# singer-yang/Aberration-Aware-Depth-from-Focus

Hardware: NVIDIA B200
Metric: focal-stack Mpix*slices/s (fused PSFNet+PSF render) (higher is better)
Workload: dtype fp16 hi/lo split, 3 terms for L1-L7, 2 terms on calibrated fp16 weights for L8, L9 and the head (worst case over any image 7.5e-5), f32 accumulate

## Files before the change

### aberration-aware-depth-from-focus_b200/csrc/aadff_api.cu

```cuda
#include <cuda_fp16.h>
#include <cuda_runtime.h>

#include <atomic>
#include <cmath>
#include <cstdio>
#include <cstring>
#include <mutex>
#include <string>
#include <vector>

#include "../../include/aadff.h"
#include "fused_tc_kernel.cuh"
#include "fused_fast2_kernel.cuh"
#include "gather_kernel.cuh"
#include "gather_coalesced_kernel.cuh"
#include "gather_strip_kernel.cuh"
#include "mlp_fp32_kernel.cuh"
#include "thinlens_kernel.cuh"
#include "focus_kernel.cuh"
#include "psf_conv_kernel.cuh"
#include "train_kernels.cuh"
#include "preprocess_kernel.cuh"
#include "spline_rotate_kernel.cuh"
#include "econ_calib.h"

using namespace aadff;

namespace {

thread_local std::string g_err;
std::atomic<long long> g_launches{0};
std::atomic<int> g_desc_swap{0};
std::atomic<int> g_dbg_flags{0};
std::atomic<unsigned long long*> g_trace{nullptr};

int fail(int code, const std::string& msg) {
    g_err = msg;
    return code;
}

template <int KS, int CN>
void launch_gc(int grid, cudaStream_t st, const float* img, const float* psf, float* out, int N, int C, int H, int W,
               int c0) {
    constexpr int smem = GatherCfg<KS>::SMEM_FLOATS(CN) * (int)sizeof(float);
    if (smem > 48 * 1024)
        cudaFuncSetAttribute(local_psf_coalesced_kernel<KS, CN>, cudaFuncAttributeMaxDynamicSharedMemorySize, smem);
    local_psf_coalesced_kernel<KS, CN><<<grid, GC_WARPS * 32, smem, st>>>(img, psf, out, N, C, H, W, c0);
}
template <int KS>
bool launch_gc_ks(int ks, int cn, int grid, cudaStream_t st, const float* img, const float* psf, float* out, int N, int C,
                  int H, int W, int c0) {
    if constexpr (KS > 31) {
        return false;
    } else {
        if (ks == KS) {
            if (cn == 3) launch_gc<KS, 3>(grid, st, img, psf, out, N, C, H, W, c0);
            else launch_gc<KS, 1>(grid, st, img, psf, out, N, C, H, W, c0);
            return true;
        }
        return launch_gc_ks<KS + 2>(ks, cn, grid, st, img, psf, out, N, C, H, W, c0);
    }
}
bool launch_gather_coalesced(int ks, int cn, int grid, cudaStream_t st, const float* img, const float* psf, float* out,
                             int N, int C, int H, int W, int c0) {
    return launch_gc_ks<3>(ks, cn, grid, st, img, psf, out, N, C, H, W, c0);
}

struct StripShape { int SL, NW, SPX; };
template <int KS> struct StripPlan;
template <> struct StripPlan<3>  { static constexpr StripShape P[3] = {{2, 7, 256}, {2, 12, 128}, {4, 16, 64}}; };
template <> struct StripPlan<5>  { static constexpr StripShape P[3] = {{1, 5, 256}, {2, 6, 128}, {2, 12, 64}}; };
template <> struct StripPlan<7>  { static constexpr StripShape P[3] = {{1, 3, 256}, {1, 6, 128}, {1, 11, 64}}; };
template <> struct StripPlan<9>  { static constexpr StripShape P[3] = {{1, 3, 128}, {1, 7, 64}, {2, 4, 64}}; };
template <> struct StripPlan<11> { static constexpr StripShape P[3] = {{1, 5, 64}, {2, 3, 64}, {2, 3, 64}}; };
template <> struct StripPlan<13> { static constexpr StripShape P[3] = {{2, 2, 64}, {1, 4, 64}, {1, 4, 64}}; };
template <> struct StripPlan<15> { static constexpr StripShape P[3] = {{1, 3, 64}, {3, 1, 64}, {3, 1, 64}}; };
constexpr int STRIP_MAX_KS = 15;

template <int KS, int CN, int SL, int NW, int SPX>
void launch_gs(int sms, cudaStream_t st, const float* img, const float* psf, float* out, int N, int C, int H, int W,
               int c0) {
    constexpr int smem = StripCfg<KS, CN, SPX>::SMEM_BYTES(SL, NW);
    static_assert(smem <= 232448, "strip gather: shared memory plan does not fit");
    if (smem > 48 * 1024)
        cudaFuncSetAttribute(local_psf_strip_kernel<KS, CN, SL, NW, SPX>, cudaFuncAttributeMaxDynamicSharedMemorySize, smem);
    const long long rows = (long long)N * ((W + SPX - 1) / SPX) * H;
    const int grid = (int)std::min<long long>((rows + NW - 1) / NW, sms);
    local_psf_strip_kernel<KS, CN, SL, NW, SPX><<<grid, NW * 32, smem, st>>>(img, psf, out, N, C, H, W, c0);
}
template <int KS, int I>
void launch_gs_plan(int cn, int sms, cudaStream_t st, const float* img, const float* psf, float* out, int N, int C, int H,
                    int W, int c0) {
    constexpr StripShape S = StripPlan<KS>::P[I];
    if (cn == 3) launch_gs<KS, 3, S.SL, S.NW, S.SPX>(sms, st, img, psf, out, N, C, H, W, c0);
    else launch_gs<KS, 1, S.SL, S.NW, S.SPX>(sms, st, img, psf, out, N, C, H, W, c0);
}
template <int KS>
bool launch_gs_ks(int ks, int cn, int plan, int sms, cudaStream_t st, const float* img, const float* psf, float* out,
                  int N, int C, int H, int W, int c0) {
    if constexpr (KS > STRIP_MAX_KS) {
        return false;
    } else {
        if (ks == KS) {
            if (plan < 0) {
                plan = 2;
                for (int i = 0; i < 3; ++i) {
                    const int spx = StripPlan<KS>::P[i].SPX;
                    if ((long long)((W + spx - 1) / spx) * spx * 10 <= (long long)W * 11 || spx <= GSW_PX) { plan = i; break; }
                }
            }
            if (plan == 1) launch_gs_plan<KS, 1>(cn, sms, st, img, psf, out, N, C, H, W, c0);
            else if (plan == 2) launch_gs_plan<KS, 2>(cn, sms, st, img, psf, out, N, C, H, W, c0);
            else launch_gs_plan<KS, 0>(cn, sms, st, img, psf, out, N, C, H, W, c0);
            return true;
        }
        return launch_gs_ks<KS + 2>(ks, cn, plan, sms, st, img, psf, out, N, C, H, W, c0);
    }
}

template <int KS>
bool launch_psf_conv(int ks, int grid, cudaStream_t st, const PsfConvArgs& a) {
    if constexpr (KS > 31) {
        return false;
    } else {
        if (ks == KS) {
            psf_conv_kernel<KS><<<grid, PC_NT, 0, st>>>(a);
            return true;
        }
        return launch_psf_conv<KS + 2>(ks, grid, st, a);
    }
}

template <int KS>
bool launch_thinlens(int ks, int grid, int smem, cudaStream_t st, const ThinLensArgs& a, const CUtensorMap& map) {
    if constexpr (KS > 31) {
        return false;
    } else {
        if (ks == KS) {
            if (smem > 48 * 1024)
                cudaFuncSetAttribute(thinlens_render_kernel<KS>, cudaFuncAttributeMaxDynamicSharedMemorySize, smem);
            thinlens_render_kernel<KS><<<grid, TL_NT, smem, st>>>(a, map);
            return true;
        }
        return launch_thinlens<KS + 2>(ks, grid, smem, st, a, map);
    }
}
template <int KS>
bool thinlens2_geometry(int ks, int cn, int* box_w, int* box_h, int* smem) {
    if constexpr (KS > 31) {
        return false;
    } else {
        if (ks == KS) {
            *box_w = ThinLens2Cfg<KS>::BW;
            *box_h = ThinLens2Cfg<KS>::HH;
            *smem = ThinLens2Cfg<KS>::SMEM_BYTES(cn);
            return true;
        }
        return thinlens2_geometry<KS + 2>(ks, cn, box_w, box_h, smem);
    }
}
template <int KS>
bool launch_thinlens2(int ks, int grid, int smem, cudaStream_t st, const ThinLensArgs& a, const CUtensorMap& map) {
    if constexpr (KS > 31) {
        return false;
    } else {
        if (ks == KS) {
            if (smem > 48 * 1024)
                cudaFuncSetAttribute(thinlens_render2_kernel<KS>, cudaFuncAttributeMaxDynamicSharedMemorySize, smem);
            thinlens_render2_kernel<KS><<<grid, TL_NT, smem, st>>>(a, map);
            return true;
        }
        return launch_thinlens2<KS + 2>(ks, grid, smem, st, a, map);
    }
}

typedef CUresult (*EncodeTiledFn)(CUtensorMap*, CUtensorMapDataType, cuuint32_t, void*, const cuuint64_t*, const cuuint64_t*,
                                  const cuuint32_t*, const cuuint32_t*, CUtensorMapInterleave, CUtensorMapSwizzle,
                                  CUtensorMapL2promotion, CUtensorMapFloatOOBfill);
EncodeTiledFn encode_tiled_fn() {
    static EncodeTiledFn fn = []() -> EncodeTiledFn {
        void* p = nullptr;
        cudaDriverEntryPointQueryResult q;
        if (cudaGetDriverEntryPoint("cuTensorMapEncodeTiled", &p, cudaEnableDefault, &q) != cudaSuccess ||
            q != cudaDriverEntryPointSuccess)
            return nullptr;
        return reinterpret_cast<EncodeTiledFn>(p);
    }();
    return fn;
}

bool make_image_map(CUtensorMap* map, const float* img, long long planes, int H, int W, int box_w, int box_h, int box_c) {
    EncodeTiledFn enc = encode_tiled_fn();
    if (!enc || (W % 4) != 0 || (reinterpret_cast<uintptr_t>(img) % 16) != 0 || box_w > 256 || box_h > 256 || box_c > 256)
        return false;
    const cuuint64_t dims[3] = {(cuuint64_t)W, (cuuint64_t)H, (cuuint64_t)planes};
    const cuuint64_t strides[2] = {(cuuint64_t)W * 4, (cuuint64_t)W * H * 4};
    const cuuint32_t box[3] = {(cuuint32_t)box_w, (cuuint32_t)box_h, (cuuint32_t)box_c};
    const cuuint32_t estr[3] = {1, 1, 1};
    return enc(map, CU_TENSOR_MAP_DATA_TYPE_FLOAT32, 3, const_cast<float*>(img), dims, strides, box, estr,
               CU_TENSOR_MAP_INTERLEAVE_NONE, CU_TENSOR_MAP_SWIZZLE_NONE, CU_TENSOR_MAP_L2_PROMOTION_L2_128B,
               CU_TENSOR_MAP_FLOAT_OOB_FILL_NONE) == CUDA_SUCCESS;
}

#define CUDA_TRY(expr)                                                                          \
    do {                                                                                        \
        cudaError_t _e = (expr);                                                                \
        if (_e != cudaSuccess)                                                                  \
            return fail(AADFF_E_CUDA, std::string(#expr) + ": " + cudaGetErrorString(_e));      \
    } while (0)

struct DeviceGuard {
    int prev = -1;
    bool ok = true;
    explicit DeviceGuard(int dev) {
        if (cudaGetDevice(&prev) != cudaSuccess) { ok = false; return; }
        if (prev != dev && cudaSetDevice(dev) != cudaSuccess) ok = false;
    }
    ~DeviceGuard() {
        if (prev >= 0) cudaSetDevice(prev);
    }
};

template <typename T>
int upload(const std::vector<T>& h, T** d) {
    CUDA_TRY(cudaMalloc(reinterpret_cast<void**>(d), h.size() * sizeof(T)));
    CUDA_TRY(cudaMemcpy(*d, h.data(), h.size() * sizeof(T), cudaMemcpyHostToDevice));
    return AADFF_OK;
}

void pack_group(const float* W, int out_f, int in_f, int n0, int N, std::vector<__half>& dst) {
    for (int kc = 0; kc < in_f / TC_SLAB_K; ++kc) {
        for (int part = 0; part < 2; ++part) {
            const size_t base = dst.size();
            dst.resize(base + (size_t)N * TC_SLAB_K);
            for (int k = 0; k < TC_SLAB_K; ++k) {
                for (int n = 0; n < N; ++n) {
                    const int row = n0 + n, col = kc * TC_SLAB_K + k;
                    const float w = (row < out_f) ? W[(size_t)row * in_f + col] : 0.0f;
                    const __half hi = __float2half_rn(w);
                    const __half v = part == 0 ? hi : __float2half_rn(w - __half2float(hi));
                    dst[base + (size_t)(k / 8) * (N * 8) + (size_t)n * 8 + (k % 8)] = v;
                }
            }
        }
    }
}

void pack_bias_slab(const float* bias, int N, std::vector<__half>& dst) {
    const size_t base = dst.size();
    dst.resize(base + (size_t)N * 16, __float2half_rn(0.f));
    for (int n = 0; n < N; ++n) {
        const __half hi = __float2half_rn(bias[n]);
        dst[base + (size_t)n * 8 + 0] = hi;
        dst[base + (size_t)n * 8 + 1] = __float2half_rn(bias[n] - __half2float(hi));
    }
}

}

struct aadff_psfnet {
    int device = 0, ks = 0, kk = 0, n_layers = 0;
    int num_sms = 0, smem_optin = 0;
    Fp32Net f32{};
    std::vector<float*> owned;
    bool tc_ok = false;
    std::string tc_why;
    uint8_t* d_wpack = nullptr;
    float* d_bias_tc = nullptr;
    float* d_w0b0 = nullptr;
    TcGroup groups[TC_MAX_GROUPS]{};
    uint32_t w_off_econ[TC_MAX_GROUPS]{};
    uint8_t* d_wpack_econ = nullptr;
    size_t pack_bytes = 0;
    bool econ_ready = false;
    std::mutex econ_mu;
    std::vector<std::vector<float>> host_w, host_b;
    std::vector<int> host_dims;
    int n_groups = 0, n_hidden = 0, n_bias = 0, head_bias0 = 0;
    cudaStream_t ws_stream = nullptr, ws_copy_stream = nullptr;
    std::vector<cudaEvent_t> ws_events;
    float* ws = nullptr;
    size_t ws_bytes = 0;
};

struct aadff_trainer {
    int device = 0, n_layers = 0, batch = 0, kk = 0;
    std::vector<int> dims;
    std::vector<size_t> w_off, b_off;
    size_t n_params = 0;
    float *params = nullptr, *grads = nullptr, *m = nullptr, *v = nullptr;
    std::vector<float*> act;
    float *z = nullptr, *p = nullptr, *target = nullptr, *loss = nullptr;
    std::vector<float*> dz;
    AdamHyper* hyper = nullptr;
    AdamHyper host_hyper{};
    long long step = 0;
    cudaGraph_t graph = nullptr;
    cudaGraphExec_t exec = nullptr;
    cudaStream_t cap_stream = nullptr;
    cudaStream_t side[2] = {nullptr, nullptr};
    std::vector<cudaEvent_t> evs;
};

static void trainer_free(aadff_trainer* t) {
    if (!t) return;
    DeviceGuard guard(t->device);
    if (t->exec) cudaGraphExecDestroy(t->exec);
    if (t->graph) cudaGraphDestroy(t->graph);
    if (t->cap_stream) cudaStreamDestroy(t->cap_stream);
    for (cudaEvent_t ev : t->evs) cudaEventDestroy(ev);
    for (int i = 0; i < 2; ++i) if (t->side[i]) cudaStreamDestroy(t->side[i]);
    for (float* a : t->act) cudaFree(a);
    cudaFree(t->params); cudaFree(t->grads); cudaFree(t->m); cudaFree(t->v);
    cudaFree(t->z); cudaFree(t->p); cudaFree(t->target);
    for (float* d : t->dz) cudaFree(d);
    cudaFree(t->loss); cudaFree(t->hyper);
    delete t;
}

template <int EPI>
static void tg_launch(cudaStream_t st, const float* A, long long sa_i, long long sa_k, const float* B, long long sb_k,
                      long long sb_j, float* C, int M, int N, int K, const float* aux) {
    dim3 grid((N + TG_TILE - 1) / TG_TILE, (M + TG_TILE - 1) / TG_TILE);
    train_gemm_kernel<EPI><<<grid, TG_NT, 0, st>>>(A, sa_i, sa_k, B, sb_k, sb_j, C, M, N, K, aux);
}

static int trainer_record(aadff_trainer* t, cudaStream_t st) {
    const int L = t->n_layers, M = t->batch;
    cudaStream_t* side = t->side;
    size_t next_ev = 0;
    auto new_event = [&]() { return t->evs[next_ev++]; };
    for (int l = 0; l < L; ++l) {
        const int K = t->dims[l], N = t->dims[l + 1];
        const float* W = t->params + t->w_off[l];
        const float* b = t->params + t->b_off[l];
        if (l < L - 1) tg_launch<TG_BIAS_RELU>(st, t->act[l], K, 1, W, 1, K, t->act[l + 1], M, N, K, b);
        else tg_launch<TG_BIAS>(st, t->act[l], K, 1, W, 1, K, t->z, M, N, K, b);
    }
    train_head_kernel<<<(M * 32 + 255) / 256, 256, 0, st>>>(t->z, t->target, t->p, t->dz[L - 1], t->loss, M, t->kk);
    for (int l = L - 1; l >= 0; --l) {
        const int K = t->dims[l], N = t->dims[l + 1];
        const float* W = t->params + t->w_off[l];
        const float* dZ = t->dz[l];
        cudaEvent_t ready = new_event();
        cudaEventRecord(ready, st);
        cudaStreamWaitEvent(side[0], ready, 0);
        cudaStreamWaitEvent(side[1], ready, 0);
        tg_launch<TG_PLAIN>(side[0], dZ, 1, N, t->act[l], K, 1, t->grads + t->w_off[l], N, K, M, nullptr);
        train_colsum_kernel<<<(N + 255) / 256, 256, 0, side[1]>>>(dZ, t->grads + t->b_off[l], M, N);
        if (l > 0) tg_launch<TG_RELU_MASK>(st, dZ, N, 1, W, K, 1, t->dz[l - 1], M, K, N, t->act[l]);
    }
    for (int i = 0; i < 2; ++i) {
        cudaEvent_t done = new_event();
        cudaEventRecord(done, side[i]);
        cudaStreamWaitEvent(st, done, 0);
    }
    train_adamw_kernel<<<(int)std::min<size_t>((t->n_params + 255) / 256, 1184), 256, 0, st>>>(
        t->params, t->grads, t->m, t->v, (long long)t->n_params, t->hyper);
    const cudaError_t e = cudaGetLastError();
    if (e != cudaSuccess) return fail(AADFF_E_CUDA, std::string("trainer_record: ") + cudaGetErrorString(e));
    return AADFF_OK;
}


extern "C" {

int aadff_version(void) { return AADFF_VERSION; }
const char* aadff_last_error(void) { return g_err.c_str(); }
int64_t aadff_launch_count(void) { return g_launches.load(); }
int aadff_debug_set_desc_swap(int swap) {
    g_desc_swap.store(swap ? 1 : 0);
    return AADFF_OK;
}

int aadff_debug_set_trace(void* device_buffer) {
    g_trace.store(static_cast<unsigned long long*>(device_buffer));
    return AADFF_OK;
}
int aadff_debug_trace_entries(void) { return TC_TRACE_N; }
int aadff_debug_set_flags(int flags) {
    g_dbg_flags.store(flags);
    return AADFF_OK;
}

int aadff_psfnet_create(const float* const* weights, const float* const* biases, const int* dims, int n_layers,
                        int ks, int device, aadff_psfnet_t* out) {
    if (!weights || !biases || !dims || !out) return fail(AADFF_E_INVALID, "null argument");
    if (n_layers < 2 || n_layers > MAX_LAYERS) return fail(AADFF_E_INVALID, "n_layers must be in [2,16]");
    if (ks < 1 || (ks % 2) == 0) return fail(AADFF_E_INVALID, "kernel size must be odd and positive");
    if (dims[0] != 4 || dims[n_layers] != ks * ks)
        return fail(AADFF_E_INVALID, "dims must start with 4 and end with ks*ks");
    for (int l = 0; l < n_layers; ++l) {
        if (!weights[l] || !biases[l]) return fail(AADFF_E_INVALID, "null layer pointer");
        if (dims[l + 1] < 1 || (l + 1 < n_layers && (dims[l + 1] > 256 || dims[l + 1] % 8)))
            return fail(AADFF_E_INVALID, "hidden widths must be multiples of 8 and <= 256");
    }
    DeviceGuard guard(device);
    if (!guard.ok) return fail(AADFF_E_CUDA, "cannot select CUDA device " + std::to_string(device));
    cudaDeviceProp prop;
    CUDA_TRY(cudaGetDeviceProperties(&prop, device));
    if (prop.major != 10)
        return fail(AADFF_E_CUDA, "libaadff is built for sm_100a only; device is sm_" + std::to_string(prop.major) +
                                      std::to_string(prop.minor));

    aadff_psfnet* h = new aadff_psfnet();
    h->device = device;
    h->ks = ks;
    h->kk = ks * ks;
    h->n_layers = n_layers;
    h->num_sms = prop.multiProcessorCount;
    h->smem_optin = (int)prop.sharedMemPerBlockOptin;

    h->f32.n_layers = n_layers;
    h->f32.kk = h->kk;
    for (int l = 0; l < n_layers; ++l) {
        const int K = dims[l], Nf = dims[l + 1], npad = (Nf + 7) / 8 * 8;
        std::vector<float> wt((size_t)K * npad, 0.f), b(npad, 0.f);
        for (int n = 0; n < Nf; ++n) {
            b[n] = biases[l][n];
            for (int k = 0; k < K; ++k) wt[(size_t)k * npad + n] = weights[l][(size_t)n * K + k];
        }
        float *dw = nullptr, *db = nullptr;
        int rc = upload(wt, &dw);
        if (rc) { aadff_psfnet_destroy(h); return rc; }
        h->owned.push_back(dw);
        rc = upload(b, &db);
        if (rc) { aadff_psfnet_destroy(h); return rc; }
        h->owned.push_back(db);
        h->f32.wt[l] = dw;
        h->f32.bias[l] = db;
        h->f32.k[l] = K;
        h->f32.npad[l] = npad;
    }
#define CREATE_TRY(expr)                                                                         \
    do {                                                                                         \
        cudaError_t _e = (expr);                                                                 \
        if (_e != cudaSuccess) {                                                                 \
            aadff_psfnet_destroy(h);                                                             \
            return fail(AADFF_E_CUDA, std::string(#expr) + ": " + cudaGetErrorString(_e));       \
        }                                                                                        \
    } while (0)
    CREATE_TRY(cudaFuncSetAttribute(mlp_fp32_kernel<true>, cudaFuncAttributeMaxDynamicSharedMemorySize, F32_SMEM));
    CREATE_TRY(cudaFuncSetAttribute(mlp_fp32_kernel<false>, cudaFuncAttributeMaxDynamicSharedMemorySize, F32_SMEM));

    h->tc_ok = true;
    if (n_layers < 3 || dims[1] != 64) { h->tc_ok = false; h->tc_why = "first hidden width must be 64"; }
    for (int l = 2; l < n_layers && h->tc_ok; ++l)
        if (dims[l] != TC_HID) { h->tc_ok = false; h->tc_why = "hidden width must be 256"; }
    if (ks > TC_MAX_KS) { h->tc_ok = false; h->tc_why = "kernel size > 31"; }
    const int nh_pad = (h->kk + 15) / 16 * 16;
    const int n_head_blocks = (nh_pad + 255) / 256;
    if (h->tc_ok && (n_layers - 2) + n_head_blocks > TC_MAX_GROUPS) { h->tc_ok = false; h->tc_why = "too many layers"; }
    if (h->tc_ok) {
        std::vector<__half> pack;
        std::vector<float> bias_tc;
        int gi = 0;
        for (int l = 1; l < n_layers - 1; ++l, ++gi) {
            TcGroup& g = h->groups[gi];
            g.w_off = (uint32_t)(pack.size() * sizeof(__half));
            g.K = (uint16_t)dims[l];
            g.N = TC_HID;
            g.terms = 3;
            g.bias_off = (uint16_t)bias_tc.size();
            g.new_a = 1;
            g.tap0 = 0;
            pack_bias_slab(biases[l], TC_HID, pack);
            pack_group(weights[l], dims[l + 1], dims[l], 0, TC_HID, pack);
            bias_tc.insert(bias_tc.end(), biases[l], biases[l] + TC_HID);
        }
        h->n_hidden = gi;
        const int L = n_layers - 1;
        const int head_bias0 = (int)bias_tc.size();
        h->head_bias0 = head_bias0;
        bias_tc.resize(head_bias0 + nh_pad, 0.f);
        for (int n = 0; n < h->kk; ++n) bias_tc[head_bias0 + n] = -1.4426950408889634f * biases[L][n];
        for (int b = 0; b < n_head_blocks; ++b, ++gi) {
            TcGroup& g = h->groups[gi];
            const int N = std::min(256, nh_pad - 256 * b);
            g.w_off = (uint32_t)(pack.size() * sizeof(__half));
            g.K = TC_HID;
            g.N = (uint16_t)N;
            g.terms = 3;
            g.bias_off = (uint16_t)(head_bias0 + 256 * b);
            g.new_a = (b == 0);
            g.tap0 = (uint16_t)(256 * b);
            pack_group(weights[L], h->kk, TC_HID, 256 * b, N, pack);
        }
        h->n_groups = gi;
        h->n_bias = (int)bias_tc.size();
        h->host_dims.assign(dims, dims + n_layers + 1);
        for (int l = 0; l < n_layers; ++l) {
            h->host_w.emplace_back(weights[l], weights[l] + (size_t)dims[l] * dims[l + 1]);
            h->host_b.emplace_back(biases[l], biases[l] + dims[l + 1]);
        }
        h->pack_bytes = pack.size() * sizeof(__half);
        std::vector<float> w0b0(320);
        std::memcpy(w0b0.data(), weights[0], 256 * sizeof(float));
        std::memcpy(w0b0.data() + 256, biases[0], 64 * sizeof(float));
        __half* dp = nullptr;
        int rc = upload(pack, &dp);
        if (rc) { aadff_psfnet_destroy(h); return rc; }
        h->d_wpack = reinterpret_cast<uint8_t*>(dp);
        rc = upload(bias_tc, &h->d_bias_tc);
        if (rc) { aadff_psfnet_destroy(h); return rc; }
        rc = upload(w0b0, &h->d_w0b0);
        if (rc) { aadff_psfnet_destroy(h); return rc; }
        const int so = h->smem_optin;
        const auto attr = cudaFuncAttributeMaxDynamicSharedMemorySize;
        CREATE_TRY(cudaFuncSetAttribute(fused_psfnet_render_kernel<true, false, 0>, attr, so));
#define AADFF_SET_ATTR(U)                                                                        \
        CREATE_TRY(cudaFuncSetAttribute(fused_psfnet_render_kernel<false, false, U>, attr, so));   \
        CREATE_TRY(cudaFuncSetAttribute(fused_psfnet_render_kernel<false, false, U, true>, attr, so));   \
        CREATE_TRY(cudaFuncSetAttribute(fused_psfnet_render_kernel<false, true, U>, attr, so));
        AADFF_SET_ATTR(0) AADFF_SET_ATTR(1) AADFF_SET_ATTR(3) AADFF_SET_ATTR(13) AADFF_SET_ATTR(12) AADFF_SET_ATTR(15)
#undef AADFF_SET_ATTR
        CREATE_TRY(cudaFuncSetAttribute(fused_psfnet_render_kernel<false, false, 14>, attr, so));
        CREATE_TRY(cudaFuncSetAttribute(fused_psfnet_render_kernel<false, true, 14>, attr, so));
    }
#undef CREATE_TRY
    *out = h;
    return AADFF_OK;
}

int aadff_psfnet_destroy(aadff_psfnet_t h) {
    if (!h) return AADFF_OK;
    DeviceGuard guard(h->device);
    for (float* p : h->owned) cudaFree(p);
    cudaFree(h->d_wpack);
    cudaFree(h->d_wpack_econ);
    cudaFree(h->d_bias_tc);
    cudaFree(h->d_w0b0);
    cudaFree(h->ws);
    if (h->ws_stream) cudaStreamDestroy(h->ws_stream);
    if (h->ws_copy_stream) cudaStreamDestroy(h->ws_copy_stream);
    for (cudaEvent_t e : h->ws_events) cudaEventDestroy(e);
    delete h;
    return AADFF_OK;
}

static int ensure_econ(aadff_psfnet_t h) {
    std::lock_guard<std::mutex> lock(h->econ_mu);
    if (h->econ_ready) return AADFF_OK;
    const int n_layers = h->n_layers, L = n_layers - 1;
    std::vector<const float*> W(n_layers), B(n_layers);
    for (int l = 0; l < n_layers; ++l) { W[l] = h->host_w[l].data(); B[l] = h->host_b[l].data(); }
    std::vector<std::vector<float>> wq;
    calibrate_econ(W.data(), B.data(), h->host_dims.data(), n_layers, TC_ECON_FIRST_LAYER, wq);
    std::vector<__half> pack;
    for (int g2 = 0; g2 < h->n_groups; ++g2) {
        const bool hidden = g2 < h->n_hidden;
        const int l = hidden ? g2 + 1 : L;
        h->w_off_econ[g2] = h->groups[g2].w_off;
        if (l < TC_ECON_FIRST_LAYER || wq[l].empty()) continue;
        h->w_off_econ[g2] = (uint32_t)(h->pack_bytes + pack.size() * sizeof(__half));
        if (hidden) {
            pack_bias_slab(B[l], TC_HID, pack);
            pack_group(wq[l].data(), h->host_dims[l + 1], h->host_dims[l], 0, TC_HID, pack);
        } else {
            pack_group(wq[l].data(), h->kk, TC_HID, h->groups[g2].tap0, h->groups[g2].N, pack);
        }
    }
    uint8_t* d = nullptr;
    CUDA_TRY(cudaMalloc(reinterpret_cast<void**>(&d), h->pack_bytes + pack.size() * sizeof(__half)));
    cudaError_t e = cudaMemcpy(d, h->d_wpack, h->pack_bytes, cudaMemcpyDeviceToDevice);
    if (e == cudaSuccess) e = cudaMemcpy(d + h->pack_bytes, pack.data(), pack.size() * sizeof(__half), cudaMemcpyHostToDevice);
    if (e != cudaSuccess) {
        cudaFree(d);
        return fail(AADFF_E_CUDA, std::string("econ weight upload: ") + cudaGetErrorString(e));
    }
    h->d_wpack_econ = d;
    h->econ_ready = true;
    return AADFF_OK;
}

static int launch_fast2(aadff_psfnet_t h, const RenderArgs& ra, cudaStream_t st, long long tile_row0, long long tile_row1) {
    if (!h->tc_ok || h->n_groups != h->n_hidden + 1 || !(g_dbg_flags.load() & 32)) return 1;
    F2Params P{};
    P.ra = ra;
    P.wpack = h->d_wpack;
    P.bias = h->d_bias_tc;
    P.w0b0 = h->d_w0b0;
    P.n_groups = h->n_groups;
    P.n_hidden = h->n_hidden;
    P.n_bias = h->n_bias;
    P.bias_skip = h->head_bias0;
    P.kk = h->kk;
    for (int i = 0; i < h->n_groups; ++i) { P.g[i] = h->groups[i]; P.g[i].terms = 1; }
    P.tiles_x = (ra.W + TC_TILE_W - 1) / TC_TILE_W;
    P.tiles_y = (ra.H + TC_TILE_H - 1) / TC_TILE_H;
    P.n_tiles = (long long)P.tiles_x * P.tiles_y * ra.N * ra.S;
    if (tile_row1 >= 0) {
        P.tile0 = tile_row0 * P.tiles_x;
        P.n_tiles = (tile_row1 - tile_row0) * P.tiles_x;
        if (P.n_tiles <= 0) return AADFF_OK;
    }
    P.halo_pitch = TC_TILE_W + ra.ks - 1;
    P.halo_bytes = (uint32_t)(TC_TILE_H + ra.ks - 1) * P.halo_pitch * 16;
    const uint32_t bias_bytes = (uint32_t)(h->n_bias - h->head_bias0) * 4;
    P.off_stage = 2 * TC_A_PART_BYTES;
    P.off_bias = P.off_stage + F2_STAGES * TC_STAGE_BYTES;
    P.off_w0 = P.off_bias + bias_bytes;
    P.off_halo = (P.off_w0 + 320 * 4 + 15u) & ~15u;
    P.off_red = P.off_halo + 2 * P.halo_bytes;
    P.off_bar = P.off_red + 2 * TC_M * 5 * 4;
    P.off_ones = (P.off_bar + TC_BAR_BYTES + 15u) & ~15u;
    P.off_bslab = P.off_ones + 2 * TC_A_LBO;
    const uint32_t smem = P.off_bslab + 2 * TC_BSLAB_BYTES;
    if (smem > (uint32_t)h->smem_optin) return 1;
    const long long units = (P.n_tiles + 1) / 2;
    const int grid = (int)std::min<long long>(units, h->num_sms);
    cudaFuncSetAttribute(fused_fast2_kernel, cudaFuncAttributeMaxDynamicSharedMemorySize, h->smem_optin);
    fused_fast2_kernel<<<grid, TC_NT, smem, st>>>(P);
    g_launches.fetch_add(1);
    CUDA_TRY(cudaGetLastError());
    return AADFF_OK;
}

static int launch_tc(aadff_psfnet_t h, RenderArgs ra, int mode, cudaStream_t st, long long tile_row0 = 0,
                     long long tile_row1 = -1, const float* probes = nullptr, float* psf_out = nullptr,
                     long long n_probes = 0) {
    if (!h->tc_ok) return fail(AADFF_E_UNSUPPORTED, "tensor-core path unavailable: " + h->tc_why + " (use AADFF_MODE_FP32)");
    const bool econ_like = (mode == AADFF_MODE_ECON || mode == AADFF_MODE_ECON8);
    if (econ_like) {
        const int rc = ensure_econ(h);
        if (rc) return rc;
    }
    if (mode == AADFF_MODE_FAST && probes == nullptr && g_trace.load() == nullptr) {
        const int rc = launch_fast2(h, ra, st, tile_row0, tile_row1);
        if (rc <= 0) return rc;
    }
    TcParams P{};
    P.ra = ra;
    P.wpack = econ_like ? h->d_wpack_econ : h->d_wpack;
    P.bias = h->d_bias_tc;
    P.w0b0 = h->d_w0b0;
    P.n_groups = h->n_groups;
    P.n_hidden = h->n_hidden;
    P.n_bias = h->n_bias;
    P.bias_skip = h->head_bias0;
    P.kk = h->kk;
    const int econ_first_dbg = (g_dbg_flags.load() >> 16) & 15;
    const int econ_first = (econ_first_dbg > TC_ECON_FIRST_GROUP) ? econ_first_dbg : TC_ECON_FIRST_GROUP;
    for (int i = 0; i < h->n_groups; ++i) {
        P.g[i] = h->groups[i];
        const bool hidden = i < h->n_hidden;
        P.g[i].terms = (mode == AADFF_MODE_FAST) ? 1
                       : (mode == AADFF_MODE_MIXED && i >= TC_MIXED_FIRST_GROUP) ? 1
                       : (mode == AADFF_MODE_ECON && i >= econ_first) ? 2
                       : (mode == AADFF_MODE_ECON8 && i >= TC_ECON8_FIRST_GROUP) ? 2
                       : 3;
        if (econ_like && P.g[i].terms == 2 && !(g_dbg_flags.load() & 256))
            P.g[i].w_off = h->w_off_econ[i];
        (void)hidden;
    }
    P.tiles_x = (ra.W + TC_TILE_W - 1) / TC_TILE_W;
    P.tiles_y = (ra.H + TC_TILE_H - 1) / TC_TILE_H;
    P.n_tiles = (long long)P.tiles_x * P.tiles_y * ra.N * ra.S;
    if (tile_row1 >= 0) {
        P.tile0 = tile_row0 * P.tiles_x;
        P.n_tiles = (tile_row1 - tile_row0) * P.tiles_x;
        if (P.n_tiles <= 0) return AADFF_OK;
    }
    if (probes != nullptr) {
        P.probes = probes;
        P.psf_out = psf_out;
        P.n_probes = n_probes;
        P.n_tiles = (n_probes + TC_M - 1) / TC_M;
    }
    P.trace = g_trace.load();
    P.dbg = (uint32_t)g_dbg_flags.load();
    uint32_t halo_bytes = (uint32_t)(TC_TILE_H + ra.ks - 1) * TC_HALO_PITCH * 16;
    if (probes != nullptr) halo_bytes = std::max<uint32_t>(halo_bytes, 8 * 32 * 9 * 4);
    const uint32_t bias_bytes = (uint32_t)(h->n_bias - h->head_bias0) * 4;
    const uint32_t ones_bytes = 2 * TC_A_LBO;
    const uint32_t bslab_bytes = 2 * TC_BSLAB_BYTES;
    const uint32_t fixed = 2 * TC_A_PART_BYTES + bias_bytes + 320 * 4 + halo_bytes + TC_M * 5 * 4 + TC_BAR_BYTES + ones_bytes +
                           bslab_bytes + 16;
    int stages = 4;
    while (stages >= 2 && fixed + (uint32_t)stages * TC_STAGE_BYTES > (uint32_t)h->smem_optin) --stages;
    if (stages < 2) return fail(AADFF_E_UNSUPPORTED, "shared memory budget exceeded for this kernel size / channel count");
    bool any_lo = false;
    for (int i = 0; i < h->n_groups; ++i) any_lo |= (P.g[i].terms >= 2);
    P.off_stage = 2 * TC_A_PART_BYTES;
    P.off_bias = P.off_stage + stages * TC_STAGE_BYTES;
    P.off_w0 = P.off_bias + bias_bytes;
    P.off_halo = P.off_w0 + 320 * 4;
    P.off_red = P.off_halo + halo_bytes;
    P.off_bar = P.off_red + TC_M * 5 * 4;
    P.off_ones = (P.off_bar + TC_BAR_BYTES + 15u) & ~15u;
    P.off_bslab = P.off_ones + ones_bytes;
    const uint32_t smem = P.off_bslab + bslab_bytes;
    P.kslab = (!any_lo && stages == 4) ? 2 : 1;
    P.n_stages = (P.kslab == 2) ? 4 : stages;
    int grid = (int)std::min<long long>(P.n_tiles, h->num_sms);
    bool all3 = true, all1 = true, econ_pat = true, econ8_pat = true, mixed_pat = true, aligned = (P.n_stages == 4 && P.kslab == 1);
    for (int i = 0; i < h->n_groups; ++i) {
        const int t = P.g[i].terms;
        all3 &= (t == 3);
        all1 &= (t == 1);
        econ_pat &= (t == (i < TC_ECON_FIRST_GROUP ? 3 : 2));
        econ8_pat &= (t == (i < TC_ECON8_FIRST_GROUP ? 3 : 2));
        mixed_pat &= (t == (i < TC_MIXED_FIRST_GROUP ? 3 : 1));
        aligned &= (((P.g[i].K / TC_SLAB_K) * (t == 3 ? 2 : 1)) % 4 == 0);
    }
    static_assert(TC_ECON_FIRST_GROUP == TC_ECON_FIRST_LAYER - 1, "group g holds layer g + 1");
    int uni = 0;
    if (all3 && P.kslab == 1) uni = aligned ? 13 : 3;
    else if (all1 && P.kslab == 2) uni = 1;
    else if (econ_pat && aligned) uni = 12;
    else if (econ8_pat && aligned && h->n_groups > TC_ECON8_FIRST_GROUP) uni = 14;
    else if (mixed_pat && aligned) uni = 15;
    const bool cl2 = P.probes == nullptr && P.trace == nullptr && uni != 0 && uni != 14 && (P.dbg & 8u) && h->num_sms >= 2;
    if (cl2) {
        grid = (int)std::min<long long>((P.n_tiles + 1) & ~1ll, (long long)(h->num_sms & ~1));
        cudaLaunchConfig_t cfg{};
        cfg.gridDim = dim3((unsigned)grid);
        cfg.blockDim = dim3(TC_NT);
        cfg.dynamicSmemBytes = smem;
        cfg.stream = st;
        cudaLaunchAttribute la[1];
        la[0].id = cudaLaunchAttributeClusterDimension;
        la[0].val.clusterDim.x = 2; la[0].val.clusterDim.y = 1; la[0].val.clusterDim.z = 1;
        cfg.attrs = la;
        cfg.numAttrs = 1;
        cudaError_t le = cudaSuccess;
        switch (uni) {
            case 1: le = cudaLaunchKernelEx(&cfg, fused_psfnet_render_kernel<false, false, 1, true>, P); break;
            case 3: le = cudaLaunchKernelEx(&cfg, fused_psfnet_render_kernel<false, false, 3, true>, P); break;
            case 13: le = cudaLaunchKernelEx(&cfg, fused_psfnet_render_kernel<false, false, 13, true>, P); break;
            case 12: le = cudaLaunchKernelEx(&cfg, fused_psfnet_render_kernel<false, false, 12, true>, P); break;
            default: le = cudaLaunchKernelEx(&cfg, fused_psfnet_render_kernel<false, false, 15, true>, P); break;
        }
        if (le != cudaSuccess) return fail(AADFF_E_CUDA, std::string("cluster launch: ") + cudaGetErrorString(le));
    } else if (P.trace != nullptr && P.probes == nullptr) {
        fused_psfnet_render_kernel<true, false, 0><<<grid, TC_NT, smem, st>>>(P);
    } else {
#define AADFF_LAUNCH(U)                                                                                   \
        case U:                                                                                           \
            if (P.probes != nullptr) fused_psfnet_render_kernel<false, true, U><<<grid, TC_NT, smem, st>>>(P);   \
            else fused_psfnet_render_kernel<false, false, U><<<grid, TC_NT, smem, st>>>(P);               \
            break;
        switch (uni) {
            AADFF_LAUNCH(1) AADFF_LAUNCH(3) AADFF_LAUNCH(13) AADFF_LAUNCH(12) AADFF_LAUNCH(14) AADFF_LAUNCH(15)
            default:
                if (P.probes != nullptr) fused_psfnet_render_kernel<false, true, 0><<<grid, TC_NT, smem, st>>>(P);
                else fused_psfnet_render_kernel<false, false, 0><<<grid, TC_NT, smem, st>>>(P);
        }
#undef AADFF_LAUNCH
    }
    g_launches.fetch_add(1);
    CUDA_TRY(cudaGetLastError());
    return AADFF_OK;
}

static int render_stack_impl(aadff_psfnet_t h, const float* img, const float* depth, const float* foc, int foc_stride,
                             float* out, const int64_t out_strides[5], int N, int C, int S, int H, int W, float d_min,
                             float d_max, int mode, void* stream, long long tile_row0 = 0, long long tile_row1 = -1);

int aadff_tile_row_height(void) { return TC_TILE_H; }
int aadff_econ_first_group(void) { return TC_ECON_FIRST_GROUP; }

int aadff_render_stack_rows_f32(aadff_psfnet_t h, const float* img, const float* depth, const float* foc, float* out,
                                const int64_t out_strides[5], int N, int C, int S, int H, int W, float d_min,
                                float d_max, int mode, int64_t tile_row_begin, int64_t tile_row_end, void* stream) {
    const long long total = (long long)N * S * ((H + TC_TILE_H - 1) / TC_TILE_H);
    if (tile_row_begin < 0 || tile_row_end < tile_row_begin || tile_row_end > total)
        return fail(AADFF_E_INVALID, "tile-row range outside [0, N*S*ceil(H/8)]");
    return render_stack_impl(h, img, depth, foc, S, out, out_strides, N, C, S, H, W, d_min, d_max, mode, stream,
                             tile_row_begin, tile_row_end);
}

int aadff_render_stack_f32(aadff_psfnet_t h, const float* img, const float* depth, const float* foc, float* out,
                           const int64_t out_strides[5], int N, int C, int S, int H, int W, float d_min,
                           float d_max, int mode, void* stream) {
    return render_stack_impl(h, img, depth, foc, S, out, out_strides, N, C, S, H, W, d_min, d_max, mode, stream);
}

static int render_stack_impl(aadff_psfnet_t h, const float* img, const float* depth, const float* foc, int foc_stride,
                             float* out, const int64_t out_strides[5], int N, int C, int S, int H, int W, float d_min,
                             float d_max, int mode, void* stream, long long tile_row0, long long tile_row1) {
    if (!h || !img || !depth || !foc || !out || !out_strides) return fail(AADFF_E_INVALID, "null argument");
    if (N < 0 || C < 1 || S < 1 || H < 1 || W < 1) return fail(AADFF_E_INVALID, "bad shape");
    if (mode < 0 || mode > 5) return fail(AADFF_E_INVALID, "unknown mode");
    if (d_max == d_min) return fail(AADFF_E_INVALID, "d_max == d_min");
    if (N == 0) return AADFF_OK;
    DeviceGuard guard(h->device);
    if (!guard.ok) return fail(AADFF_E_CUDA, "cannot select device");
    cudaStream_t st = static_cast<cudaStream_t>(stream);
    RenderArgs ra{};
    ra.img = img; ra.depth = depth; ra.foc = foc; ra.out = out;
    ra.os_n = out_strides[0]; ra.os_c = out_strides[1]; ra.os_s = out_strides[2];
    ra.os_h = out_strides[3]; ra.os_w = out_strides[4];
    ra.N = N; ra.S = S; ra.H = H; ra.W = W; ra.ks = h->ks; ra.Ctot = C;
    ra.foc_stride = foc_stride;
    ra.d_min = d_min;
    ra.d_range = d_max - d_min;
    ra.step_x = (W > 1) ? (1.0f - (-1.0f)) / (float)(W - 1) : 0.f;
    ra.step_y = (H > 1) ? (-1.0f - 1.0f) / (float)(H - 1) : 0.f;
    for (int c0 = 0; c0 < C; c0 += 4) {
        ra.c0 = c0;
        ra.C = std::min(4, C - c0);
        if (mode == AADFF_MODE_FP32) {
            long long M0 = 0, M = (long long)N * S * H * W;
            if (tile_row1 >= 0) {
                const long long tiles_y = (H + TC_TILE_H - 1) / TC_TILE_H;
                auto flat_row = [&](long long R) { return (R / tiles_y) * H + std::min<long long>((R % tiles_y) * TC_TILE_H, H); };
                M0 = flat_row(tile_row0) * W;
                M = flat_row(tile_row1) * W;
            }
            if (M > M0) {
                const int grid = (int)std::min<long long>((M - M0 + F32_TP - 1) / F32_TP, (long long)h->num_sms * 8);
                mlp_fp32_kernel<true><<<grid, F32_NT, F32_SMEM, st>>>(h->f32, ra, nullptr, nullptr, M0, M);
                g_launches.fetch_add(1);
                CUDA_TRY(cudaGetLastError());
            }
        } else {
            int rc = launch_tc(h, ra, mode, st, tile_row0, tile_row1);
            if (rc) return rc;
        }
    }
    return AADFF_OK;
}

int aadff_render_stack_host_f32(aadff_psfnet_t h, const float* img, const float* depth, const float* foc,
                                float* out, int N, int C, int S, int H, int W, float d_min, float d_max, int mode) {
    if (!h || !img || !depth || !foc || !out) return fail(AADFF_E_INVALID, "null argument");
    if (N < 1 || C < 1 || S < 1 || H < 1 || W < 1) return fail(AADFF_E_INVALID, "bad shape");
    DeviceGuard guard(h->device);
    if (!guard.ok) return fail(AADFF_E_CUDA, "cannot select device");
    const size_t n_img = (size_t)N * C * H * W, n_dep = (size_t)N * H * W, n_foc = (size_t)N * S;
    const size_t n_out = n_img * S;
    auto up = [](size_t n) { return (n + 63) / 64 * 64; };
    const size_t need = (up(n_img) + up(n_dep) + up(n_foc) + up(n_out)) * sizeof(float);
    if (!h->ws_stream) CUDA_TRY(cudaStreamCreateWithFlags(&h->ws_stream, cudaStreamNonBlocking));
    if (need > h->ws_bytes) {
        if (h->ws) CUDA_TRY(cudaFree(h->ws));
        h->ws = nullptr;
        h->ws_bytes = 0;
        CUDA_TRY(cudaMalloc(reinterpret_cast<void**>(&h->ws), need));
        h->ws_bytes = need;
    }
    float* d_img = h->ws;
    float* d_dep = d_img + up(n_img);
    float* d_foc = d_dep + up(n_dep);
    float* d_out = d_foc + up(n_foc);
    cudaStream_t st = h->ws_stream;
    CUDA_TRY(cudaMemcpyAsync(d_img, img, n_img * sizeof(float), cudaMemcpyHostToDevice, st));
    CUDA_TRY(cudaMemcpyAsync(d_dep, depth, n_dep * sizeof(float), cudaMemcpyHostToDevice, st));
    CUDA_TRY(cudaMemcpyAsync(d_foc, foc, n_foc * sizeof(float), cudaMemcpyHostToDevice, st));
    const int64_t strides[5] = {(int64_t)C * S * H * W, (int64_t)S * H * W, (int64_t)H * W, W, 1};
    if (!h->ws_copy_stream) CUDA_TRY(cudaStreamCreateWithFlags(&h->ws_copy_stream, cudaStreamNonBlocking));
    if (h->ws_events.size() < (size_t)S) {
        const size_t old = h->ws_events.size();
        h->ws_events.resize(S);
        for (size_t i = old; i < (size_t)S; ++i) CUDA_TRY(cudaEventCreateWithFlags(&h->ws_events[i], cudaEventDisableTiming));
    }
    const size_t plane = (size_t)H * W * sizeof(float);
    for (int s = 0; s < S; ++s) {
        int rc = render_stack_impl(h, d_img, d_dep, d_foc + s, S, d_out + (size_t)s * H * W, strides, N, C, 1, H, W, d_min,
                                   d_max, mode, st);
        if (rc) return rc;
        CUDA_TRY(cudaEventRecord(h->ws_events[s], st));
        CUDA_TRY(cudaStreamWaitEvent(h->ws_copy_stream, h->ws_events[s], 0));
        for (int n = 0; n < N; ++n) {
            const size_t off = ((size_t)n * C * S + s) * H * W;
            CUDA_TRY(cudaMemcpy2DAsync(out + off, (size_t)S * plane, d_out + off, (size_t)S * plane, plane, C,
                                       cudaMemcpyDeviceToHost, h->ws_copy_stream));
        }
    }
    CUDA_TRY(cudaStreamSynchronize(h->ws_copy_stream));
    CUDA_TRY(cudaStreamSynchronize(st));
    return AADFF_OK;
}

int aadff_psfnet_pred_f32(aadff_psfnet_t h, const float* inp, float* psf, int64_t M, void* stream) {
    if (!h || !inp || !psf) return fail(AADFF_E_INVALID, "null argument");
    if (M < 0) return fail(AADFF_E_INVALID, "negative M");
    if (M == 0) return AADFF_OK;
    DeviceGuard guard(h->device);
    if (!guard.ok) return fail(AADFF_E_CUDA, "cannot select device");
    RenderArgs ra{};
    ra.ks = h->ks;
    const int grid = (int)std::min<long long>((M + F32_TP - 1) / F32_TP, (long long)h->num_sms * 8);
    mlp_fp32_kernel<false><<<grid, F32_NT, F32_SMEM, static_cast<cudaStream_t>(stream)>>>(h->f32, ra, inp, psf, 0, M);
    g_launches.fetch_add(1);
    CUDA_TRY(cudaGetLastError());
    return AADFF_OK;
}

int aadff_psfnet_pred_tc_f32(aadff_psfnet_t h, const float* inp, float* psf, int64_t M, int mode, void* stream) {
    if (!h || !inp || !psf) return fail(AADFF_E_INVALID, "null argument");
    if (M < 0) return fail(AADFF_E_INVALID, "negative M");
    if (mode == AADFF_MODE_FP32) return aadff_psfnet_pred_f32(h, inp, psf, M, stream);
    if (mode < 0 || mode > 5) return fail(AADFF_E_INVALID, "unknown mode");
    if (reinterpret_cast<uintptr_t>(inp) % 16) return fail(AADFF_E_INVALID, "inp must be 16-byte aligned");
    if (M == 0) return AADFF_OK;
    DeviceGuard guard(h->device);
    if (!guard.ok) return fail(AADFF_E_CUDA, "cannot select device");
    RenderArgs ra{};
    ra.ks = h->ks; ra.N = 1; ra.S = 1; ra.H = 1; ra.W = 1; ra.C = 1; ra.Ctot = 1;
    return launch_tc(h, ra, mode, static_cast<cudaStream_t>(stream), 0, -1, inp, psf, (long long)M);
}

int aadff_local_psf_render_f32(const float* img, const float* psf, float* out, int N, int C, int H, int W, int ks,
                               void* stream) {
    if (!img || !psf || !out) return fail(AADFF_E_INVALID, "null argument");
    if (N < 0 || C < 1 || H < 1 || W < 1) return fail(AADFF_E_INVALID, "bad shape");
    if (ks < 1 || (ks % 2) == 0) return fail(AADFF_E_INVALID, "kernel size must be odd and positive");
    if (N == 0) return AADFF_OK;
    int dev = 0, sms = 0;
    CUDA_TRY(cudaGetDevice(&dev));
    CUDA_TRY(cudaDeviceGetAttribute(&sms, cudaDevAttrMultiProcessorCount, dev));
    cudaStream_t st = static_cast<cudaStream_t>(stream);
    const int dbg = g_dbg_flags.load();
    if (ks >= 3 && ks <= STRIP_MAX_KS && !(dbg & (128 | 512)) && W % 4 == 0 && reinterpret_cast<uintptr_t>(psf) % 16 == 0 &&
        reinterpret_cast<uintptr_t>(out) % 8 == 0 && (long long)N * H * ((W + 31) / 32) < (1ll << 40)) {
        int c0 = 0;
        while (c0 < C) {
            const int cn = (C - c0 >= 3) ? 3 : 1;
            if (!launch_gs_ks<3>(ks, cn, (dbg & 1024) ? 1 : (dbg & 4096) ? 2 : (dbg & 8192) ? 0 : -1, sms, st, img, psf, out, N, C, H, W, c0))
                return fail(AADFF_E_INVALID, "unsupported kernel size");
            g_launches.fetch_add(1);
            CUDA_TRY(cudaGetLastError());
            c0 += cn;
        }
        return AADFF_OK;
    }
    if (ks >= 3 && ks <= 31 && !(g_dbg_flags.load() & 128)) {
        const long long tiles = (long long)N * ((H + GC_WARPS - 1) / GC_WARPS) * ((W + GC_TW - 1) / GC_TW);
        if (tiles >= (1ll << 31)) return fail(AADFF_E_INVALID, "image batch too large for one launch");
        const int grid = (int)std::min<long long>(tiles, sms);
        int c0 = 0;
        while (c0 < C) {
            const int cn = (C - c0 >= 3) ? 3 : 1;
            if (!launch_gather_coalesced(ks, cn, grid, st, img, psf, out, N, C, H, W, c0))
                return fail(AADFF_E_INVALID, "unsupported kernel size");
            g_launches.fetch_add(1);
            CUDA_TRY(cudaGetLastError());
            c0 += cn;
        }
        return AADFF_OK;
    }
    const int kk = ks * ks;
    int P = 32;
    while (P > 4 && P * kk * 4 > GS_BUF_BYTES) P >>= 1;
    const bool stream_ok = (W % 4 == 0) && (reinterpret_cast<uintptr_t>(psf) % 16 == 0) && (P * kk * 4 <= GS_BUF_BYTES);
    if (stream_ok) {
        const int nbuf = (P == 32 && (g_dbg_flags.load() & 64)) ? 2 : 1;
        const int nw = (nbuf == 2) ? GS_TILE_H_2BUF : GS_TILE_H_1BUF;
        const int buf_bytes = (P * kk * 4 + 127) / 128 * 128;
        const int HH = nw + ks - 1, pitch = (GS_TILE_W + ks - 1) | 1;
        const int smem = nw * nbuf * buf_bytes + GS_MAXC * HH * pitch * 4 + 16 * nw;
        if (smem > 48 * 1024) {
            if (nw == GS_TILE_H_1BUF)
                CUDA_TRY(cudaFuncSetAttribute(local_psf_stream_kernel<GS_TILE_H_1BUF>,
                                              cudaFuncAttributeMaxDynamicSharedMemorySize, smem));
            else
                CUDA_TRY(cudaFuncSetAttribute(local_psf_stream_kernel<GS_TILE_H_2BUF>,
                                              cudaFuncAttributeMaxDynamicSharedMemorySize, smem));
        }
        const long long tiles = (long long)N * ((H + nw - 1) / nw) * ((W + GS_TILE_W - 1) / GS_TILE_W);
        const int grid = (int)std::min<long long>(tiles, sms);
        for (int c0 = 0; c0 < C; c0 += GS_MAXC) {
            const int cn = std::min(GS_MAXC, C - c0);
            if (nw == GS_TILE_H_1BUF)
                local_psf_stream_kernel<GS_TILE_H_1BUF><<<grid, nw * 32, smem, st>>>(img, psf, out, N, C, H, W, ks, c0, cn,
                                                                                   P, nbuf, buf_bytes);
            else
                local_psf_stream_kernel<GS_TILE_H_2BUF><<<grid, nw * 32, smem, st>>>(img, psf, out, N, C, H, W, ks, c0, cn,
                                                                                   P, nbuf, buf_bytes);
            g_launches.fetch_add(1);
            CUDA_TRY(cudaGetLastError());
        }
        return AADFF_OK;
    }
    const int smem = GATHER_WARPS * 32 * (GATHER_TT + 1) * (int)sizeof(float);
    if (smem > 48 * 1024)
        CUDA_TRY(cudaFuncSetAttribute(local_psf_render_kernel, cudaFuncAttributeMaxDynamicSharedMemorySize, smem));
    const long long items = (long long)N * H * ((W + 31) / 32);
    const int grid = (int)std::min<long long>((items + GATHER_WARPS - 1) / GATHER_WARPS, (long long)sms * 3);
    for (int c0 = 0; c0 < C; c0 += GATHER_MAXC) {
        local_psf_render_kernel<<<grid, GATHER_WARPS * 32, smem, st>>>(img, psf, out, N, C, H, W, ks, c0,
                                                                       std::min(GATHER_MAXC, C - c0));
        g_launches.fetch_add(1);
        CUDA_TRY(cudaGetLastError());
    }
    return AADFF_OK;
}

int aadff_any_negative_f32(const float* x, int64_t n, unsigned char* flag_dev, void* stream) {
    if (!x || !flag_dev || n < 0) return fail(AADFF_E_INVALID, "bad argument");
    cudaStream_t st = static_cast<cudaStream_t>(stream);
    CUDA_TRY(cudaMemsetAsync(flag_dev, 0, 1, st));
    if (n == 0) return AADFF_OK;
    const int grid = (int)std::min<long long>((n + 255) / 256, 592);
    any_negative_kernel<<<grid, 256, 0, st>>>(x, (long long)n, flag_dev);
    g_launches.fetch_add(1);
    CUDA_TRY(cudaGetLastError());
    return AADFF_OK;
}

int aadff_thinlens_render_f32(const float* img, const float* depth, const float* foc, float* out, int N, int C, int H,
                              int W, int ks, float foc_len, float fnum, float pixel_size, float d_lo, float d_hi,
                              int flip_sign, const unsigned char* flip_sign_dev, void* stream) {
    if (!img || !depth || !foc || !out) return fail(AADFF_E_INVALID, "null argument");
    if (N < 0 || C < 1 || H < 1 || W < 1) return fail(AADFF_E_INVALID, "bad shape");
    if (ks < 1 || (ks % 2) == 0) return fail(AADFF_E_INVALID, "kernel size must be odd and positive");
    if (!(fnum > 0.f) || !(pixel_size > 0.f) || !(d_hi > d_lo)) return fail(AADFF_E_INVALID, "bad lens parameters");
    if (N == 0) return AADFF_OK;
    int dev = 0, sms = 0, optin = 0;
    CUDA_TRY(cudaGetDevice(&dev));
    CUDA_TRY(cudaDeviceGetAttribute(&sms, cudaDevAttrMultiProcessorCount, dev));
    CUDA_TRY(cudaDeviceGetAttribute(&optin, cudaDevAttrMaxSharedMemoryPerBlockOptin, dev));
    ThinLensArgs a{};
    a.img = img; a.depth = depth; a.foc = foc; a.out = out;
    a.N = N; a.C = C; a.H = H; a.W = W;
    a.k1 = (float)((double)foc_len / (double)fnum);
    a.foc_len = foc_len; a.ps = pixel_size; a.d_lo = d_lo; a.d_hi = d_hi; a.flip = flip_sign ? 1 : 0;
    a.flip_dev = flip_sign_dev;
    if (ks > 31) return fail(AADFF_E_UNSUPPORTED, "thin-lens kernel sizes above 31 are not built");
    cudaStream_t st = static_cast<cudaStream_t>(stream);
    const bool two_px = !(g_dbg_flags.load() & 2048);
    const int tl_r = (ks - 1) / 2, tl_sh = (4 - tl_r % 4) % 4;
    const int tile_w = two_px ? TL2_TILE_W : TL_TILE_W;
    const long long tiles = (long long)N * ((H + TL_TILE_H - 1) / TL_TILE_H) * ((W + tile_w - 1) / tile_w);
    if (tiles >= (1ll << 31)) return fail(AADFF_E_INVALID, "image batch too large for one launch");
    const int grid = (int)std::min<long long>(tiles, (long long)sms * 4);
    for (int c0 = 0; c0 < C; c0 += TL_MAXC) {
        a.c0 = c0;
        a.cn = std::min(TL_MAXC, C - c0);
        int HH = TL_TILE_H + ks - 1, BW = (TL_TILE_W + ks - 1 + tl_sh + 3) / 4 * 4;
        int smem = (ks <= 15 ? 2 : 1) * ((a.cn * HH * BW + 31) / 32 * 32) * 4 + 128;
        if (two_px && !thinlens2_geometry<1>(ks, a.cn, &BW, &HH, &smem)) return fail(AADFF_E_INVALID, "unsupported kernel size");
        if (smem > optin) return fail(AADFF_E_UNSUPPORTED, "kernel size too large for the shared-memory halo tile");
        CUtensorMap map;
        std::memset(&map, 0, sizeof(map));
        a.use_tma = make_image_map(&map, img, (long long)N * C, H, W, BW, HH, a.cn) && !(g_dbg_flags.load() & 16);
        const bool launched = two_px ? launch_thinlens2<1>(ks, grid, smem, st, a, map) : launch_thinlens<1>(ks, grid, smem, st, a, map);
        if (!launched) return fail(AADFF_E_INVALID, "unsupported kernel size");
        g_launches.fetch_add(1);
        CUDA_TRY(cudaGetLastError());
    }
    return AADFF_OK;
}

int aadff_render_psf_map_f32(const float* img, const float* psf_map, float* out, int B, int C, int H, int W, int ks,
                             int grid, const int* row_bounds, const int* col_bounds, void* stream) {
    if (!img || !psf_map || !out || !row_bounds || !col_bounds) return fail(AADFF_E_INVALID, "null argument");
    if (B < 0 || C < 1 || H < 1 || W < 1) return fail(AADFF_E_INVALID, "bad shape");
    if (ks < 1 || ks > 31 || (ks % 2) == 0) return fail(AADFF_E_INVALID, "PSF kernel size should be odd (and <= 31)");
    if (grid < 1 || grid > PC_MAX_GRID) return fail(AADFF_E_INVALID, "grid must be in [1, 32]");
    if ((ks - 1) / 2 >= H || (ks - 1) / 2 >= W) return fail(AADFF_E_INVALID, "reflect padding needs (ks-1)/2 < H, W");
    if (B == 0) return AADFF_OK;
    PsfConvArgs a{};
    a.img = img; a.psf_map = psf_map; a.out = out;
    a.B = B; a.C = C; a.H = H; a.W = W; a.grid = grid;
    for (int i = 0; i <= grid; ++i) { a.hb[i] = row_bounds[i]; a.wb[i] = col_bounds[i]; }
    if (a.hb[0] != 0 || a.wb[0] != 0 || a.hb[grid] > H || a.wb[grid] > W) return fail(AADFF_E_INVALID, "bad patch bounds");
    for (int i = 0; i < grid; ++i) {
        if (a.hb[i + 1] < a.hb[i] || a.wb[i + 1] < a.wb[i]) return fail(AADFF_E_INVALID, "patch bounds must ascend");
        a.max_ch = std::max(a.max_ch, a.hb[i + 1] - a.hb[i]);
        a.max_cw = std::max(a.max_cw, a.wb[i + 1] - a.wb[i]);
    }
    if (a.max_ch == 0 || a.max_cw == 0) return AADFF_OK;
    int dev = 0, sms = 0;
    CUDA_TRY(cudaGetDevice(&dev));
    CUDA_TRY(cudaDeviceGetAttribute(&sms, cudaDevAttrMultiProcessorCount, dev));
    const long long tiles = (long long)B * C * grid * grid * ((a.max_ch + PC_TILE_H - 1) / PC_TILE_H) *
                            ((a.max_cw + PC_TILE_W - 1) / PC_TILE_W);
    const int nblk = (int)std::min<long long>(tiles, (long long)sms * 8);
    if (!launch_psf_conv<1>(ks, nblk, static_cast<cudaStream_t>(stream), a)) return fail(AADFF_E_INVALID, "unsupported kernel size");
    g_launches.fetch_add(1);
    CUDA_TRY(cudaGetLastError());
    return AADFF_OK;
}

int aadff_preprocess_rgbd_u8(const uint8_t* bgr, const uint16_t* depth, float* aif_out, float* depth_out, int B, int H, int W,
                             int h, int w, float depth_div, int depth_mode, const float* jitter, const uint8_t* flips,
                             void* stream) {
    if ((!bgr && !depth) || (bgr && !aif_out) || (depth && !depth_out)) return fail(AADFF_E_INVALID, "null argument");
    if (B < 0 || H < 1 || W < 1 || h < 1 || w < 1) return fail(AADFF_E_INVALID, "bad shape");
    if (depth && !(depth_div > 0.f)) return fail(AADFF_E_INVALID, "depth divisor must be positive");
    if (depth_mode != 0 && depth_mode != 1) return fail(AADFF_E_INVALID, "depth_mode must be 0 (antialias) or 1 (cv2 linear)");
    if (B == 0) return AADFF_OK;
    PreprocessArgs a{};
    a.bgr = bgr; a.depth = depth; a.aif_out = bgr ? aif_out : nullptr; a.depth_out = depth ? depth_out : nullptr;
    a.jitter = jitter; a.flips = flips;
    a.B = B; a.H = H; a.W = W; a.h = h; a.w = w; a.depth_div = depth_div; a.depth_mode = depth_mode;
    const long long per_image = (long long)h * w;
    const dim3 grid((unsigned)std::min<long long>((per_image + 255) / 256, 148 * 16), (unsigned)B);
    if (B > 65535) return fail(AADFF_E_INVALID, "batch too large for one launch");
    preprocess_rgbd_kernel<false><<<grid, 256, 0, static_cast<cudaStream_t>(stream)>>>(a);
    g_launches.fetch_add(1);
    CUDA_TRY(cudaGetLastError());
    return AADFF_OK;
}

int aadff_prepare_planes_u8(const uint8_t* bgr, const uint16_t* depth, float* planes, int B, int H, int W, float depth_div,
                            const float* jitter, const uint8_t* flips, void* stream) {
    if ((!bgr && !depth) || !planes) return fail(AADFF_E_INVALID, "null argument");
    if (B < 0 || H < 1 || W < 1) return fail(AADFF_E_INVALID, "bad shape");
    if (depth && !(depth_div > 0.f)) return fail(AADFF_E_INVALID, "depth divisor must be positive");
    if (B > 65535) return fail(AADFF_E_INVALID, "batch too large for one launch");
    if (B == 0) return AADFF_OK;
    PlanesArgs a{};
    a.bgr = bgr; a.depth = depth; a.planes = planes; a.jitter = jitter; a.flips = flips;
    a.B = B; a.H = H; a.W = W; a.P = (bgr ? 3 : 0) + (depth ? 1 : 0); a.depth_div = depth_div;
    const dim3 grid((unsigned)std::min<long long>(((long long)H * W + 255) / 256, 148 * 8), (unsigned)B);
    prepare_planes_kernel<<<grid, 256, 0, static_cast<cudaStream_t>(stream)>>>(a);
    g_launches.fetch_add(1);
    CUDA_TRY(cudaGetLastError());
    return AADFF_OK;
}

int aadff_spline_affine_f32(const float* planes, float* work, float* out, int B, int P, int H, int W, const double* xform,
                            int clamp_plane, void* stream) {
    if (!planes || !work || !out || !xform) return fail(AADFF_E_INVALID, "null argument");
    if (B < 0 || P < 1 || H < 1 || W < 1) return fail(AADFF_E_INVALID, "bad shape");
    if (clamp_plane >= P) return fail(AADFF_E_INVALID, "clamp_plane out of range");
    if (B > 65535) return fail(AADFF_E_INVALID, "batch too large for one launch");
    if (B == 0) return AADFF_OK;
    cudaStream_t st = static_cast<cudaStream_t>(stream);
    const long long n = (long long)B * P * H * W;
    float* tmp = work;
    float* coef = work + n;
    const unsigned blocks = (unsigned)std::min<long long>((n + 255) / 256, 148 * 16);
    spline_prefilter_kernel<1><<<blocks, 256, 0, st>>>(planes, tmp, (long long)B * P, H, W);
    spline_prefilter_kernel<0><<<blocks, 256, 0, st>>>(tmp, coef, (long long)B * P, H, W);
    AffineArgs a{};
    a.coef = coef; a.raw = planes; a.out = out; a.xform = xform; a.B = B; a.P = P; a.H = H; a.W = W; a.clamp_plane = clamp_plane;
    const dim3 grid((unsigned)std::min<long long>(((long long)H * W + 255) / 256, 148 * 8), (unsigned)B);
    spline_affine_kernel<<<grid, 256, 0, st>>>(a);
    g_launches.fetch_add(3);
    CUDA_TRY(cudaGetLastError());
    return AADFF_OK;
}

int aadff_resize_planes_f32(const float* planes, float* aif_out, float* depth_out, int B, int P, int H, int W, int h, int w,
                            int depth_mode, void* stream) {
    if (!planes || (!aif_out && !depth_out)) return fail(AADFF_E_INVALID, "null argument");
    if (B < 0 || H < 1 || W < 1 || h < 1 || w < 1) return fail(AADFF_E_INVALID, "bad shape");
    if (P != (aif_out ? 3 : 0) + (depth_out ? 1 : 0)) return fail(AADFF_E_INVALID, "P must be 3 (image), 1 (depth) or 4 (both)");
    if (depth_mode != 0 && depth_mode != 1) return fail(AADFF_E_INVALID, "depth_mode must be 0 (antialias) or 1 (cv2 linear)");
    if (B > 65535) return fail(AADFF_E_INVALID, "batch too large for one launch");
    if (B == 0) return AADFF_OK;
    PreprocessArgs a{};
    a.aif_out = aif_out; a.depth_out = depth_out; a.fsrc = planes; a.fsrc_planes = P; a.fsrc_depth_plane = P - 1;
    a.B = B; a.H = H; a.W = W; a.h = h; a.w = w; a.depth_div = 1.f; a.depth_mode = depth_mode;
    const long long per_image = (long long)h * w;
    const dim3 grid((unsigned)std::min<long long>((per_image + 255) / 256, 148 * 16), (unsigned)B);
    preprocess_rgbd_kernel<true><<<grid, 256, 0, static_cast<cudaStream_t>(stream)>>>(a);
    g_launches.fetch_add(1);
    CUDA_TRY(cudaGetLastError());
    return AADFF_OK;
}

int aadff_select_focus_f32(const float* depth_m, int B, int64_t HW, int num, float* out, void* stream) {
    if (!depth_m || !out) return fail(AADFF_E_INVALID, "null argument");
    if (B < 0 || HW < 1) return fail(AADFF_E_INVALID, "bad shape");
    if (num <= 3) return fail(AADFF_E_INVALID, "Focal stack size is too small");
    if (B == 0) return AADFF_OK;
    select_focus_kernel<<<B, FOCUS_NT, 0, static_cast<cudaStream_t>(stream)>>>(depth_m, (long long)HW, num, out);
    g_launches.fetch_add(1);
    CUDA_TRY(cudaGetLastError());
    return AADFF_OK;
}


int aadff_trainer_create(const float* const* weights, const float* const* biases, const int* dims, int n_layers,
                         int batch, float beta1, float beta2, float eps, float weight_decay, int device,
                         aadff_trainer_t* out) {
    if (!weights || !biases || !dims || !out) return fail(AADFF_E_INVALID, "null argument");
    if (n_layers < 1 || n_layers > MAX_LAYERS || batch < 1) return fail(AADFF_E_INVALID, "bad n_layers / batch");
    DeviceGuard guard(device);
    if (!guard.ok) return fail(AADFF_E_CUDA, "cannot select CUDA device " + std::to_string(device));
    aadff_trainer* t = new aadff_trainer();
    t->device = device; t->n_layers = n_layers; t->batch = batch; t->kk = dims[n_layers];
    t->dims.assign(dims, dims + n_layers + 1);
    t->host_hyper.beta1 = beta1; t->host_hyper.beta2 = beta2; t->host_hyper.eps = eps; t->host_hyper.weight_decay = weight_decay;
    size_t off = 0;
    int wmax = 0;
    for (int l = 0; l < n_layers; ++l) {
        t->w_off.push_back(off); off += (size_t)dims[l] * dims[l + 1];
        t->b_off.push_back(off); off += (size_t)dims[l + 1];
        wmax = std::max(wmax, std::max(dims[l], dims[l + 1]));
    }
    t->n_params = off;
#define TR_TRY(expr)                                                                             \
    do {                                                                                         \
        cudaError_t _e = (expr);                                                                 \
        if (_e != cudaSuccess) {                                                                 \
            trainer_free(t);                                                                     \
            return fail(AADFF_E_CUDA, std::string(#expr) + ": " + cudaGetErrorString(_e));       \
        }                                                                                        \
    } while (0)
    auto dalloc = [&](float** p, size_t n) { return cudaMalloc(reinterpret_cast<void**>(p), n * sizeof(float)); };
    TR_TRY(dalloc(&t->params, off)); TR_TRY(dalloc(&t->grads, off)); TR_TRY(dalloc(&t->m, off)); TR_TRY(dalloc(&t->v, off));
    TR_TRY(cudaMemset(t->m, 0, off * sizeof(float))); TR_TRY(cudaMemset(t->v, 0, off * sizeof(float)));
    for (int l = 0; l < n_layers; ++l) {
        if (!weights[l] || !biases[l]) { trainer_free(t); return fail(AADFF_E_INVALID, "null layer pointer"); }
        TR_TRY(cudaMemcpy(t->params + t->w_off[l], weights[l], (size_t)dims[l] * dims[l + 1] * sizeof(float), cudaMemcpyHostToDevice));
        TR_TRY(cudaMemcpy(t->params + t->b_off[l], biases[l], (size_t)dims[l + 1] * sizeof(float), cudaMemcpyHostToDevice));
        float* a = nullptr;
        TR_TRY(dalloc(&a, (size_t)batch * dims[l]));
        t->act.push_back(a);
    }
    TR_TRY(dalloc(&t->z, (size_t)batch * t->kk)); TR_TRY(dalloc(&t->p, (size_t)batch * t->kk));
    TR_TRY(dalloc(&t->target, (size_t)batch * t->kk));
    for (int l = 0; l < n_layers; ++l) {
        float* d = nullptr;
        TR_TRY(dalloc(&d, (size_t)batch * dims[l + 1]));
        t->dz.push_back(d);
    }
    (void)wmax;
    TR_TRY(dalloc(&t->loss, 1));
    TR_TRY(cudaMalloc(reinterpret_cast<void**>(&t->hyper), sizeof(AdamHyper)));
    TR_TRY(cudaStreamCreateWithFlags(&t->cap_stream, cudaStreamNonBlocking));
    for (int i = 0; i < 2; ++i) TR_TRY(cudaStreamCreateWithFlags(&t->side[i], cudaStreamNonBlocking));
    for (int i = 0; i < n_layers + 2; ++i) {
        cudaEvent_t ev = nullptr;
        TR_TRY(cudaEventCreateWithFlags(&ev, cudaEventDisableTiming));
        t->evs.push_back(ev);
    }
    TR_TRY(cudaStreamBeginCapture(t->cap_stream, cudaStreamCaptureModeThreadLocal));
    const int rc = trainer_record(t, t->cap_stream);
    cudaError_t ce = cudaStreamEndCapture(t->cap_stream, &t->graph);
    if (rc != AADFF_OK || ce != cudaSuccess) { trainer_free(t); return rc ? rc : fail(AADFF_E_CUDA, std::string("graph capture: ") + cudaGetErrorString(ce)); }
    TR_TRY(cudaGraphInstantiate(&t->exec, t->graph, 0));
#undef TR_TRY
    *out = t;
    return AADFF_OK;
}

int aadff_trainer_destroy(aadff_trainer_t t) {
    trainer_free(t);
    return AADFF_OK;
}

int aadff_trainer_step(aadff_trainer_t t, const float* inp, const float* target, float lr, float* loss_out, void* stream) {
    if (!t || !inp || !target) return fail(AADFF_E_INVALID, "null argument");
    DeviceGuard guard(t->device);
    if (!guard.ok) return fail(AADFF_E_CUDA, "cannot select device");
    cudaStream_t st = static_cast<cudaStream_t>(stream);
    const size_t M = (size_t)t->batch;
    CUDA_TRY(cudaMemcpyAsync(t->act[0], inp, M * t->dims[0] * sizeof(float), cudaMemcpyDeviceToDevice, st));
    CUDA_TRY(cudaMemcpyAsync(t->target, target, M * t->kk * sizeof(float), cudaMemcpyDeviceToDevice, st));
    t->step += 1;
    AdamHyper h = t->host_hyper;
    h.lr = lr;
    h.bias_correction1 = (float)(1.0 - std::pow((double)h.beta1, (double)t->step));
    h.bias_correction2_sqrt = (float)std::sqrt(1.0 - std::pow((double)h.beta2, (double)t->step));
    train_hyper_kernel<<<1, 1, 0, st>>>(t->hyper, h, t->loss);
    CUDA_TRY(cudaGraphLaunch(t->exec, st));
    g_launches.fetch_add(2 + 3 * t->n_layers * 2);
    if (loss_out) CUDA_TRY(cudaMemcpyAsync(loss_out, t->loss, sizeof(float), cudaMemcpyDeviceToDevice, st));
    CUDA_TRY(cudaGetLastError());
    return AADFF_OK;
}

int aadff_trainer_read(aadff_trainer_t t, int which, float* const* weights, float* const* biases, void* stream) {
    if (!t || !weights) return fail(AADFF_E_INVALID, "null argument");
    DeviceGuard guard(t->device);
    if (!guard.ok) return fail(AADFF_E_CUDA, "cannot select device");
    cudaStream_t st = static_cast<cudaStream_t>(stream);
    CUDA_TRY(cudaStreamSynchronize(st));
    if (which == 2) {
        CUDA_TRY(cudaMemcpy(weights[0], t->p, (size_t)t->batch * t->kk * sizeof(float), cudaMemcpyDeviceToHost));
        return AADFF_OK;
    }
    if (which != 0 && which != 1) return fail(AADFF_E_INVALID, "which must be 0, 1 or 2");
    if (!biases) return fail(AADFF_E_INVALID, "null argument");
    const float* src = which == 0 ? t->params : t->grads;
    for (int l = 0; l < t->n_layers; ++l) {
        CUDA_TRY(cudaMemcpy(weights[l], src + t->w_off[l], (size_t)t->dims[l] * t->dims[l + 1] * sizeof(float), cudaMemcpyDeviceToHost));
        CUDA_TRY(cudaMemcpy(biases[l], src + t->b_off[l], (size_t)t->dims[l + 1] * sizeof(float), cudaMemcpyDeviceToHost));
    }
    return AADFF_OK;
}

int aadff_debug_umma_gemm(const float* A, const float* B, float* D, int K, int N, int device) {
    if (!A || !B || !D) return fail(AADFF_E_INVALID, "null argument");
    if (K < 32 || K > 256 || K % 32 || N < 16 || N > 256 || N % 16) return fail(AADFF_E_INVALID, "bad K/N");
    DeviceGuard guard(device);
    if (!guard.ok) return fail(AADFF_E_CUDA, "cannot select device");
    std::vector<__half> pack_all, pack_hi;
    pack_group(B, N, K, 0, N, pack_all);
    for (int kc = 0; kc < K / TC_SLAB_K; ++kc)
        pack_hi.insert(pack_hi.end(), pack_all.begin() + (size_t)(2 * kc) * N * TC_SLAB_K,
                       pack_all.begin() + (size_t)(2 * kc + 1) * N * TC_SLAB_K);
    float *dA = nullptr, *dD = nullptr;
    __half* dB = nullptr;
    CUDA_TRY(cudaMalloc(reinterpret_cast<void**>(&dA), (size_t)128 * K * 4));
    CUDA_TRY(cudaMalloc(reinterpret_cast<void**>(&dD), (size_t)128 * N * 4));
    CUDA_TRY(cudaMalloc(reinterpret_cast<void**>(&dB), pack_hi.size() * 2));
    CUDA_TRY(cudaMemcpy(dA, A, (size_t)128 * K * 4, cudaMemcpyHostToDevice));
    CUDA_TRY(cudaMemcpy(dB, pack_hi.data(), pack_hi.size() * 2, cudaMemcpyHostToDevice));
    const int smem = TC_A_PART_BYTES + 131072 + 64;
    CUDA_TRY(cudaFuncSetAttribute(debug_umma_gemm_kernel, cudaFuncAttributeMaxDynamicSharedMemorySize, smem));
    debug_umma_gemm_kernel<<<1, 128, smem>>>(dA, reinterpret_cast<const uint8_t*>(dB), dD, K, N,
                                             (uint32_t)g_desc_swap.load());
    g_launches.fetch_add(1);
    CUDA_TRY(cudaGetLastError());
    CUDA_TRY(cudaDeviceSynchronize());
    CUDA_TRY(cudaMemcpy(D, dD, (size_t)128 * N * 4, cudaMemcpyDeviceToHost));
    cudaFree(dA); cudaFree(dB); cudaFree(dD);
    return AADFF_OK;
}


int aadff_debug_econ_round(const float* W, int N, int K, const float* A, int NC, float* out) {
    if (!W || !A || !out || N < 1 || K < 1 || NC < 1) return fail(AADFF_E_INVALID, "bad args");
    std::vector<float> a(A, A + (size_t)NC * K), q;
    if (!gptq_round_fp16(W, N, K, a, NC, q)) return fail(AADFF_E_INVALID, "activation covariance is not positive definite");
    std::memcpy(out, q.data(), q.size() * sizeof(float));
    return AADFF_OK;
}

int aadff_debug_mma_timing(const int* mmas_per_commit, int n_patterns, int reps, int N, int epi_load,
                           uint64_t* out_cycles, int device) {
    if (!mmas_per_commit || !out_cycles || n_patterns < 1 || n_patterns > 16) return fail(AADFF_E_INVALID, "bad args");
    DeviceGuard guard(device);
    if (!guard.ok) return fail(AADFF_E_CUDA, "cannot select device");
    int* d_m = nullptr;
    unsigned long long* d_out = nullptr;
    CUDA_TRY(cudaMalloc(reinterpret_cast<void**>(&d_m), n_patterns * sizeof(int)));
    CUDA_TRY(cudaMalloc(reinterpret_cast<void**>(&d_out), 64 * sizeof(unsigned long long)));
    CUDA_TRY(cudaMemcpy(d_m, mmas_per_commit, n_patterns * sizeof(int), cudaMemcpyHostToDevice));
    uint8_t* d_src = nullptr;
    CUDA_TRY(cudaMalloc(reinterpret_cast<void**>(&d_src), 65536));
    CUDA_TRY(cudaMemset(d_src, 0, 65536));
    CUDA_TRY(cudaMemset(d_out, 0, 64 * sizeof(unsigned long long)));
    const int smem = TC_A_PART_BYTES + 65536 + 128;
    CUDA_TRY(cudaFuncSetAttribute(debug_mma_timing_kernel, cudaFuncAttributeMaxDynamicSharedMemorySize, smem));
    debug_mma_timing_kernel<<<1, 128, smem>>>(d_out, n_patterns, d_m, reps, N, epi_load, d_src);
    CUDA_TRY(cudaGetLastError());
    CUDA_TRY(cudaDeviceSynchronize());
    CUDA_TRY(cudaMemcpy(out_cycles, d_out, 64 * sizeof(unsigned long long), cudaMemcpyDeviceToHost));
    cudaFree(d_src);
    cudaFree(d_m);
    cudaFree(d_out);
    return AADFF_OK;
}

}
```

### aberration-aware-depth-from-focus_b200/csrc/fused_tc_kernel.cuh

```cuda
#pragma once
#include <cuda_fp16.h>
#include <cuda_runtime.h>
#include "ptx_sm100.cuh"
#include "render_args.h"

namespace aadff {

constexpr int TC_TILE_H = 8;
constexpr int TC_TILE_W = 16;
constexpr int TC_M = TC_TILE_H * TC_TILE_W;
constexpr int TC_HALO_PITCH = 48;
constexpr int TC_HID = 256;
constexpr int TC_SLAB_K = 32;
constexpr int TC_STAGE_BYTES = TC_HID * TC_SLAB_K * 2;
constexpr int TC_A_PART_BYTES = TC_M * TC_HID * 2;
constexpr int TC_A_LBO = TC_M * 16;
constexpr int TC_EPI_WARPS = 8;
constexpr int TC_EPI_THREADS = TC_EPI_WARPS * 32;
constexpr int TC_NT = 64 + TC_EPI_THREADS;
constexpr int TC_MAX_GROUPS = 16;
constexpr int TC_MAX_STAGES = 8;
constexpr int TC_MAX_KS = 31;
constexpr int TC_MAX_C = 4;
constexpr int TC_BAR_BYTES = 256;
constexpr int TC_BSLAB_BYTES = TC_HID * 16;
constexpr int TC_TRACE_N = 4096;
constexpr int TC_MIXED_FIRST_GROUP = 3;
constexpr int TC_ECON_FIRST_GROUP = 4;
constexpr int TC_ECON8_FIRST_GROUP = 7;

struct TcGroup {
    uint32_t w_off;
    uint16_t K;
    uint16_t N;
    uint16_t terms;
    uint16_t bias_off;
    uint16_t new_a;
    uint16_t tap0;
};

struct TcParams {
    RenderArgs ra;
    const uint8_t* wpack;
    const float* bias;
    const float* w0b0;
    TcGroup g[TC_MAX_GROUPS];
    int n_groups, n_hidden;
    int n_bias, n_stages, kk;
    int bias_skip;
    int kslab;
    int tiles_x, tiles_y;
    long long n_tiles;
    long long tile0;
    uint32_t off_stage, off_bias, off_w0, off_halo, off_red, off_bar, off_ones;
    uint32_t off_bslab;
    uint32_t dbg;
    const float* probes;
    float* psf_out;
    long long n_probes;
    unsigned long long* trace;
};

template <bool ON>
struct TcTrace {
    unsigned long long* p;
    int n;
    __device__ __forceinline__ void init(unsigned long long* base, int role) {
        if (ON) {
            p = (base != nullptr && blockIdx.x == 0) ? base + role * TC_TRACE_N : nullptr;
            n = 0;
        }
    }
    __device__ __forceinline__ void ev(unsigned code) {
        if (ON) {
            if (p != nullptr && n < TC_TRACE_N)
                p[n++] = ((unsigned long long)code << 40) | ((unsigned long long)clock64() & 0xFFFFFFFFFFull);
        }
    }
};

__device__ __forceinline__ uint64_t tc_desc(uint32_t addr, uint32_t lbo, uint32_t sbo, uint32_t swap) {
    return swap ? umma_smem_desc(addr, sbo, lbo) : umma_smem_desc(addr, lbo, sbo);
}

__device__ __forceinline__ uint32_t pack_half2(float a, float b) {
    __half2 h = __floats2half2_rn(a, b);
    return *reinterpret_cast<uint32_t*>(&h);
}

__device__ __forceinline__ uint32_t pack_half2_relu(float a, float b) {
    uint32_t r;
    asm("cvt.rn.relu.f16x2.f32 %0, %1, %2;" : "=r"(r) : "f"(b), "f"(a));
    return r;
}

__device__ __forceinline__ uint32_t pack_half2_relu_rz(float a, float b) {
    uint32_t r;
    asm("cvt.rz.relu.f16x2.f32 %0, %1, %2;" : "=r"(r) : "f"(b), "f"(a));
    return r;
}

__device__ __forceinline__ void store_split8(const float (&v)[8], uint32_t addr_hi, uint32_t addr_lo, bool need_lo) {
    uint32_t h[4];
#pragma unroll
    for (int u = 0; u < 4; ++u) h[u] = pack_half2(v[2 * u], v[2 * u + 1]);
    st_shared_v4(addr_hi, h[0], h[1], h[2], h[3]);
    if (need_lo) {
        uint32_t l[4];
#pragma unroll
        for (int u = 0; u < 4; ++u) {
            const float2 f = __half22float2(*reinterpret_cast<__half2*>(&h[u]));
            l[u] = pack_half2(v[2 * u] - f.x, v[2 * u + 1] - f.y);
        }
        st_shared_v4(addr_lo, l[0], l[1], l[2], l[3]);
    }
}

__device__ __forceinline__ void epi_group8(const uint32_t* acc, uint32_t a_hi, uint32_t a_lo,
                                           uint32_t kg, uint32_t a_row, bool need_lo) {
    if (!need_lo) {
        uint32_t h[4];
#pragma unroll
        for (int u = 0; u < 4; ++u) h[u] = pack_half2_relu(__uint_as_float(acc[2 * u]), __uint_as_float(acc[2 * u + 1]));
        st_shared_v4(a_hi + kg * TC_A_LBO + a_row, h[0], h[1], h[2], h[3]);
        return;
    }
    uint32_t h[4], l[4];
#pragma unroll
    for (int u = 0; u < 4; ++u) {
        const float a0 = __uint_as_float(acc[2 * u]), a1 = __uint_as_float(acc[2 * u + 1]);
        h[u] = pack_half2_relu_rz(a0, a1);
        const float2 f = __half22float2(*reinterpret_cast<__half2*>(&h[u]));
        l[u] = pack_half2_relu(a0 - f.x, a1 - f.y);
    }
    const uint32_t off = kg * TC_A_LBO + a_row;
    st_shared_v4(a_hi + off, h[0], h[1], h[2], h[3]);
    st_shared_v4(a_lo + off, l[0], l[1], l[2], l[3]);
}

constexpr int TC_WARP_PRODUCER = TC_EPI_WARPS;
constexpr int TC_WARP_MMA = TC_EPI_WARPS + 1;

template <bool TRACE, bool PRED, int UNI, bool CL2 = false>
__global__ void __launch_bounds__(TC_NT, 1) fused_psfnet_render_kernel(const __grid_constant__ TcParams P) {
    static_assert(!(CL2 && (PRED || TRACE)), "the cluster variant exists for the render kernels only");
    constexpr int UM = UNI % 10;
    const uint32_t cta_rank = CL2 ? cluster_ctarank() : 0u;
    const long long first_tile = CL2 ? (long long)(blockIdx.x & ~1u) : (long long)blockIdx.x;
    const long long my_iters = (P.n_tiles > first_tile) ? (P.n_tiles - first_tile + gridDim.x - 1) / gridDim.x : 0;
    constexpr bool ALIGNED = UNI >= 10;
    const int kslab_c = (UM == 3 || UM == 2 || UM == 4 || UM == 5) ? 1 : UM == 1 ? 2 : P.kslab;
    auto terms_of = [&](int gi) -> int {
        return UM == 3 ? 3 : UM == 1 ? 1 : UM == 2 ? (gi < TC_ECON_FIRST_GROUP ? 3 : 2)
                                         : UM == 4 ? (gi < TC_ECON8_FIRST_GROUP ? 3 : 2)
                                         : UM == 5 ? (gi < TC_MIXED_FIRST_GROUP ? 3 : 1) : (int)P.g[gi].terms;
    };
    extern __shared__ __align__(1024) uint8_t smem[];
    const uint32_t sbase = smem_u32(smem);
    const int warp = threadIdx.x >> 5, lane = threadIdx.x & 31;
    const RenderArgs& ra = P.ra;

    const uint32_t a_hi = sbase, a_lo = sbase + TC_A_PART_BYTES;
    const uint32_t stage0 = sbase + P.off_stage;
    const int stage_bytes = kslab_c * TC_STAGE_BYTES, stages_in_area = 4 / kslab_c;
    auto stage_addr = [&](int st) {
        return st < stages_in_area ? stage0 + st * stage_bytes : a_lo + (st - stages_in_area) * stage_bytes;
    };
    float* s_bias = reinterpret_cast<float*>(smem + P.off_bias);
    float* s_w0 = reinterpret_cast<float*>(smem + P.off_w0);
    float4* s_halo = reinterpret_cast<float4*>(smem + P.off_halo);
    float* s_red = reinterpret_cast<float*>(smem + P.off_red);
    const uint32_t bar0 = sbase + P.off_bar;
    auto bar_full = [&](int s) { return bar0 + 8u * s; };
    auto bar_empty = [&](int s) { return bar0 + 8u * (TC_MAX_STAGES + s); };
    auto bar_aready = [&](int j) { return bar0 + 8u * (2 * TC_MAX_STAGES + j); };
    auto bar_accfull = [&](int b) { return bar0 + 8u * (2 * TC_MAX_STAGES + 8 + b); };
    auto bar_accfree = [&](int b) { return bar0 + 8u * (2 * TC_MAX_STAGES + 10 + b); };
    auto bar_bfull = [&]() { return bar0 + 8u * (2 * TC_MAX_STAGES + 12); };
    auto bar_bempty = [&]() { return bar0 + 8u * (2 * TC_MAX_STAGES + 13); };
    volatile uint32_t* tmem_slot = reinterpret_cast<volatile uint32_t*>(smem + P.off_bar + 8 * (2 * TC_MAX_STAGES + 14));
    static_assert(8 * (2 * TC_MAX_STAGES + 14) + 4 <= TC_BAR_BYTES, "barrier area too small");

    if (threadIdx.x == 0) {
        for (int s = 0; s < TC_MAX_STAGES; ++s) { mbar_init(bar_full(s), 1); mbar_init(bar_empty(s), CL2 ? 2 : 1); }
        for (int j = 0; j < 8; ++j)
            mbar_init(bar_aready(j), (kslab_c == 2 || j < 4) ? TC_EPI_WARPS : 2 * TC_EPI_WARPS);
        for (int b = 0; b < 2; ++b) { mbar_init(bar_accfull(b), 1); mbar_init(bar_accfree(b), TC_EPI_WARPS); }
        mbar_init(bar_bfull(), 1);
        mbar_init(bar_bempty(), 1);
        fence_mbar_init();
    }
    for (int i = threadIdx.x; i < P.n_bias - P.bias_skip; i += TC_NT) s_bias[i] = __ldg(P.bias + P.bias_skip + i);
    for (int i = threadIdx.x; i < 2 * TC_M; i += TC_NT) {
        uint4 v = make_uint4(0u, 0u, 0u, 0u);
        if (i < TC_M) v.x = 0x3C003C00u;
        *reinterpret_cast<uint4*>(smem + P.off_ones + (i < TC_M ? 0 : TC_A_LBO) + (i % TC_M) * 16) = v;
    }
    for (int i = threadIdx.x; i < TC_BSLAB_BYTES / 16; i += TC_NT)
        *reinterpret_cast<uint4*>(smem + P.off_bslab + TC_BSLAB_BYTES + i * 16) = make_uint4(0u, 0u, 0u, 0u);
    fence_proxy_async_smem();
    for (int i = threadIdx.x; i < 320; i += TC_NT) s_w0[i] = __ldg(P.w0b0 + i);
    if (warp == TC_WARP_PRODUCER) tmem_alloc<512>(smem_u32(const_cast<uint32_t*>(tmem_slot)));
    tc_fence_before_sync();
    __syncthreads();
    tc_fence_after_sync();
    const uint32_t tmem_base = *tmem_slot;
    if (CL2) cluster_sync_all();

    if (warp == TC_WARP_PRODUCER) {
        int stage = 0;
        uint32_t phase = 0, bphase = 0;
        TcTrace<TRACE> tr; tr.init(lane == 0 ? P.trace : nullptr, 0);
        auto ring_copy = [&](uint32_t dst, const uint8_t* src, uint32_t bytes, uint32_t bar) {
            if (CL2) {
                const uint32_t half = bytes >> 1;
                bulk_g2s_multicast(dst + cta_rank * half, src + cta_rank * half, half, bar, (uint16_t)3);
            } else {
                bulk_g2s(dst, src, bytes, bar);
            }
        };
        for (long long iter = 0; iter < my_iters; ++iter) {
            for (int gi = 0; gi < P.n_groups; ++gi) {
                const uint32_t bytes = (uint32_t)P.g[gi].N * (TC_SLAB_K * 2);
                const int nparts = (terms_of(gi) == 3) ? 2 : 1;
                const uint8_t* src = P.wpack + P.g[gi].w_off;
                const int kslab = kslab_c;
                const int nit = P.g[gi].K / (TC_SLAB_K * kslab);
                if (gi < P.n_hidden) {
                    mbar_wait(bar_bempty(), bphase ^ 1);
                    if (elect_one_sync()) {
                        if (P.dbg & 1) {
                            mbar_arrive(bar_bfull());
                        } else {
                            mbar_arrive_expect_tx(bar_bfull(), TC_BSLAB_BYTES);
                            bulk_g2s(sbase + P.off_bslab, src, TC_BSLAB_BYTES, bar_bfull());
                        }
                    }
                    __syncwarp();
                    bphase ^= 1;
                    src += (uint32_t)P.g[gi].N * 32;
                }
                for (int it = 0; it < nit; ++it) {
                    uint32_t pair_bar = 0;
                    for (int part = 0; part < nparts; ++part) {
                        mbar_wait(bar_empty(stage), phase ^ 1);
                        tr.ev(0x100 + gi);
                        if (part == 0) pair_bar = bar_full(stage);
                        if (elect_one_sync()) {
                            if (P.dbg & 1) {
                                if (!(nparts == 2 && P.n_stages >= 4 && part == 1)) mbar_arrive(bar_full(stage));
                            } else if (nparts == 2 && P.n_stages >= 4) {
                                if (part == 0) mbar_arrive_expect_tx(pair_bar, 2 * bytes);
                                ring_copy(stage_addr(stage), src + (size_t)(it * 2 + part) * bytes, bytes, pair_bar);
                            } else {
                                mbar_arrive_expect_tx(bar_full(stage), bytes * kslab);
                                for (int hs = 0; hs < kslab; ++hs)
                                    ring_copy(stage_addr(stage) + hs * TC_STAGE_BYTES,
                                              src + (size_t)((it * kslab + hs) * 2 + part) * bytes, bytes, bar_full(stage));
                            }
                        }
                        __syncwarp();
                        if (++stage == P.n_stages) { stage = 0; phase ^= 1; }
                    }
                }
            }
        }
    } else if (warp == TC_WARP_MMA) {
        int stage = 0;
        uint32_t fbits = 0, aphase = 0, frphase = 0;
        uint32_t bphase = 0;
        uint32_t gcount = 0;
        TcTrace<TRACE> tr; tr.init(lane == 0 ? P.trace : nullptr, 1);
        const uint64_t da_hi = umma_smem_desc(a_hi, TC_A_LBO, 128);
        const uint64_t da_lo = umma_smem_desc(a_lo, TC_A_LBO, 128);
        const uint64_t da_ones = umma_smem_desc(sbase + P.off_ones, TC_A_LBO, 128);
        constexpr uint32_t KSTEP_A = (2 * TC_A_LBO) >> 4;
        constexpr uint32_t STAGE_STEP = TC_STAGE_BYTES >> 4;
        auto release = [&](uint32_t bar) {
            if (CL2) umma_commit_multicast(bar, (uint16_t)3);
            else umma_commit(bar);
        };
        for (long long iter = 0; iter < my_iters; ++iter) {
            for (int gi = 0; gi < P.n_groups; ++gi) {
                const uint32_t gN = P.g[gi].N;
                const int nkc = P.g[gi].K / TC_SLAB_K;
                const bool three = terms_of(gi) == 3;
                const bool use_al = terms_of(gi) >= 2;
                const bool new_a = P.g[gi].new_a != 0;
                const uint32_t buf = gcount & 1;
                if (gcount >= 2) {
                    mbar_wait(bar_accfree(buf), (frphase >> buf) & 1);
                    frphase ^= 1u << buf;
                }
                tc_fence_after_sync();
                tr.ev(0x200 + gi);
                const uint32_t d_tmem = tmem_base + buf * 256;
                const uint32_t idesc = umma_idesc_f16_f32(TC_M, gN);
                const uint32_t kstep_b = (2 * gN * 16) >> 4;
                const uint64_t db0 = umma_smem_desc(stage0, gN * 16, 128);
                const int kslab = kslab_c;
                const int nit = P.g[gi].K / (TC_SLAB_K * kslab);
                const bool has_bias = gi < P.n_hidden;
                if (has_bias) {
                    mbar_wait(bar_bfull(), bphase);
                    bphase ^= 1;
                    tc_fence_after_sync();
                    if (elect_one_sync()) {
                        umma_f16_ss(d_tmem, da_ones, umma_smem_desc(sbase + P.off_bslab, TC_BSLAB_BYTES, 128), idesc, 0);
                        umma_commit(bar_bempty());
                    }
                    __syncwarp();
                }
                bool pre_waited = false;
                auto kstep = [&](const int it) {
                    const int kc = it * kslab;
                    const uint64_t ah = da_hi + (uint32_t)kc * (2 * KSTEP_A);
                    const uint64_t al = da_lo + (uint32_t)kc * (2 * KSTEP_A);
                    if (ALIGNED) stage = (three ? 2 * it : it) & 3;
                    if (!pre_waited) {
                        tr.ev(0x500 + kc);
                        { mbar_wait(bar_full(stage), (fbits >> stage) & 1); fbits ^= 1u << stage; }
                        tr.ev(0x600 + kc);
                        if (new_a && (kslab == 2 || it < 3 || it == 4)) {
                            mbar_wait(bar_aready(it), (aphase >> it) & 1);
                            aphase ^= 1u << it;
                            tr.ev(0x400 + kc);
                        }
                    }
                    tc_fence_after_sync();
                    const int hi_stage = stage;
                    const bool last = (it + 1 == nit);
                    auto next_stage = [&](int st) { return ALIGNED ? ((st + 1) & 3) : (st + 1 == P.n_stages ? 0 : st + 1); };
                    if (use_al) {
                        stage = next_stage(stage);
                        const bool merged = three && (ALIGNED || P.n_stages >= 4);
                        if (elect_one_sync()) {
                            const uint64_t db = (db0 & ~0x3FFFull) | ((stage_addr(hi_stage) & 0x3FFFFu) >> 4);
                            umma_f16_ss(d_tmem, ah, db, idesc, has_bias || it != 0);
                            umma_f16_ss(d_tmem, ah + KSTEP_A, db + kstep_b, idesc, 1);
                            umma_f16_ss(d_tmem, al, db, idesc, 1);
                            umma_f16_ss(d_tmem, al + KSTEP_A, db + kstep_b, idesc, 1);
                            if (!three) {
                                if (last) umma_commit(bar_accfull(buf));
                                release(bar_empty(hi_stage));
                            } else {
                                release(bar_empty(hi_stage));
                                if (merged) {
                                    const uint64_t dl = (db0 & ~0x3FFFull) | ((stage_addr(stage) & 0x3FFFFu) >> 4);
                                    umma_f16_ss(d_tmem, ah, dl, idesc, 1);
                                    umma_f16_ss(d_tmem, ah + KSTEP_A, dl + kstep_b, idesc, 1);
                                    if (last) umma_commit(bar_accfull(buf));
                                    release(bar_empty(stage));
                                }
                            }
                        }
                        __syncwarp();
                        if (three) {
                            if (!merged) {
                                { mbar_wait(bar_full(stage), (fbits >> stage) & 1); fbits ^= 1u << stage; }
                                tc_fence_after_sync();
                                if (elect_one_sync()) {
                                    const uint64_t dl = (db0 & ~0x3FFFull) | ((stage_addr(stage) & 0x3FFFFu) >> 4);
                                    umma_f16_ss(d_tmem, ah, dl, idesc, 1);
                                    umma_f16_ss(d_tmem, ah + KSTEP_A, dl + kstep_b, idesc, 1);
                                    if (last) umma_commit(bar_accfull(buf));
                                    release(bar_empty(stage));
                                }
                                __syncwarp();
                            }
                            stage = next_stage(stage);
                        }
                        return;
                    }
                    if (elect_one_sync()) {
                        const uint64_t db = (db0 & ~0x3FFFull) | ((stage_addr(hi_stage) & 0x3FFFFu) >> 4);
                        umma_f16_ss(d_tmem, ah, db, idesc, has_bias || it != 0);
                        umma_f16_ss(d_tmem, ah + KSTEP_A, db + kstep_b, idesc, 1);
                        if (kslab == 2) {
                            umma_f16_ss(d_tmem, ah + 2 * KSTEP_A, db + STAGE_STEP, idesc, 1);
                            umma_f16_ss(d_tmem, ah + 3 * KSTEP_A, db + STAGE_STEP + kstep_b, idesc, 1);
                        }
                    }
                    __syncwarp();
                    stage = next_stage(stage);
                    pre_waited = false;
                    if (it + 1 < nit) {
                        tr.ev(0x500 + kc + kslab);
                        { mbar_wait(bar_full(stage), (fbits >> stage) & 1); fbits ^= 1u << stage; }
                        if (new_a && (kslab == 2 || it + 1 < 3 || it + 1 == 4)) {
                            mbar_wait(bar_aready(it + 1), (aphase >> (it + 1)) & 1);
                            aphase ^= 1u << (it + 1);
                        }
                        tr.ev(0x400 + kc + kslab);
                        pre_waited = true;
                    }
                    if (elect_one_sync()) {
                        if (last) umma_commit(bar_accfull(buf));
                        release(bar_empty(hi_stage));
                    }
                    __syncwarp();
                };
                if (nit == 8) {
#pragma unroll
                    for (int it = 0; it < 8; ++it) kstep(it);
                } else if (nit == 4) {
#pragma unroll
                    for (int it = 0; it < 4; ++it) kstep(it);
                } else {
                    for (int it = 0; it < nit; ++it) kstep(it);
                }
                tr.ev(0x700 + gi);
                ++gcount;
            }
        }
    } else {
        const int e = warp;
        const int q = warp & 3;
        const int hh = e >> 2;
        const int et = e * 32 + lane;
        const int row = q * 32 + lane;
        const int ty = row >> 4, tx = row & 15;
        const uint32_t t_lane = tmem_base + ((uint32_t)(q * 32) << 16);
        const int ks = ra.ks, r = (ks - 1) / 2, kk = P.kk;
        const int HH = TC_TILE_H + ks - 1, HW = TC_TILE_W + ks - 1;
        const int tiles_xy = P.tiles_x * P.tiles_y;
        const uint32_t a_row = (uint32_t)row * 16;
        uint32_t afphase = 0;
        unsigned long long gcount = 0;
        TcTrace<TRACE> tr; tr.init((lane == 0 && (e == 0 || e == 7)) ? P.trace : nullptr, e == 0 ? 2 : 3);
        const float NEG_LOG2E = -1.4426950408889634f;
        const bool fine = kslab_c == 1;
        const bool pred_one_block = PRED && (P.n_groups - P.n_hidden == 1) && (P.g[P.n_hidden].N <= 128);

        auto tile_coords = [&](long long tile, int& n, int& s, int& h0, int& w0) {
            const long long gt = tile + P.tile0;
            const int txy = (int)(gt % tiles_xy);
            const long long ns = gt / tiles_xy;
            s = (int)(ns % ra.S);
            n = (int)(ns / ra.S);
            h0 = (txy / P.tiles_x) * TC_TILE_H;
            w0 = (txy % P.tiles_x) * TC_TILE_W;
        };
        float4 nx_in = make_float4(0.f, 0.f, 0.f, 0.f);
        auto fetch_dz = [&](long long tile, float& d, float& f) {
            if (CL2 && tile >= P.n_tiles) { d = 0.f; f = 0.f; }
            if (tile < P.n_tiles) {
                if constexpr (PRED) {
                    const long long m = tile * TC_M + row;
                    nx_in = (m < P.n_probes) ? __ldg(reinterpret_cast<const float4*>(P.probes) + m)
                                             : make_float4(0.f, 0.f, 0.f, 0.f);
                } else {
                    int n, s, h0, w0;
                    tile_coords(tile, n, s, h0, w0);
                    const int hc = min(h0 + ty, ra.H - 1), wc = min(w0 + tx, ra.W - 1);
                    d = __ldg(ra.depth + ((long long)n * ra.H + hc) * ra.W + wc);
                    f = __ldg(ra.foc + (long long)n * ra.foc_stride + s);
                }
            }
        };
        float nx_depth = 0.f, nx_foc = 0.f;
        fetch_dz(blockIdx.x, nx_depth, nx_foc);

        auto layer0 = [&](long long t) {
            float x, y, z, fz;
            if constexpr (PRED) {
                x = nx_in.x; y = nx_in.y; z = nx_in.z; fz = nx_in.w;
            } else {
                int n, s, h0, w0;
                tile_coords(t, n, s, h0, w0);
                x = coord_x(min(w0 + tx, ra.W - 1), ra.W, ra.step_x);
                y = coord_y(min(h0 + ty, ra.H - 1), ra.H, ra.step_y);
                z = depth_to_z(nx_depth, ra.d_min, ra.d_range);
                fz = depth_to_z(nx_foc, ra.d_min, ra.d_range);
            }
            const bool need_lo = terms_of(0) >= 2;
#pragma unroll
            for (int i = 0; i < 4; ++i) {
                const int kg = fine ? ((i >> 1) * 4 + 2 * hh + (i & 1)) : (hh * 4 + i);
                float v[8];
#pragma unroll
                for (int u = 0; u < 8; ++u) {
                    const int f = kg * 8 + u;
                    const float4 wv = *reinterpret_cast<const float4*>(s_w0 + f * 4);
                    float a = s_w0[256 + f];
                    a = fmaf(wv.x, x, a); a = fmaf(wv.y, y, a); a = fmaf(wv.z, z, a); a = fmaf(wv.w, fz, a);
                    v[u] = fmaxf(a, 0.f);
                }
                const uint32_t off = (uint32_t)kg * TC_A_LBO + a_row;
                store_split8(v, a_hi + off, a_lo + off, need_lo);
            }
            fence_proxy_async_smem();
            __syncwarp();
            if (lane == 0) {
                if (fine) { mbar_arrive(bar_aready(0)); mbar_arrive(bar_aready(1)); }
                else mbar_arrive(bar_aready(0));
            }
        };
        if (my_iters > 0) layer0(blockIdx.x);

        long long tile = blockIdx.x;
        for (long long iter = 0; iter < my_iters; ++iter, tile += gridDim.x) {
            const bool dummy = CL2 && tile >= P.n_tiles;
            int n = 0, s = 0, h0 = 0, w0 = 0;
            if constexpr (!PRED) tile_coords(dummy ? 0 : tile, n, s, h0, w0);
            const int h = h0 + ty, w = w0 + tx;
            const long long m_row = tile * TC_M + row;
            const bool valid = PRED ? (m_row < P.n_probes) : ((h < ra.H) && (w < ra.W) && !dummy);
            tr.ev(0x800);
            fetch_dz(tile + gridDim.x, nx_depth, nx_foc);

            named_bar_sync(1, TC_EPI_THREADS);
            const float* img_n = ra.img + ((long long)n * ra.Ctot + ra.c0) * ra.H * ra.W;
            const long long cstride = (long long)ra.H * ra.W;
            auto halo_fetch = [&](int idx, float4& v) -> int {
                if (PRED || dummy || idx >= HH * HW) return -1;
                const int yy = idx / HW, xx = idx - yy * HW;
                const int gy = min(max(h0 + yy - r, 0), ra.H - 1), gx = min(max(w0 + xx - r, 0), ra.W - 1);
                const float* px = img_n + (long long)gy * ra.W + gx;
                v.x = __ldg(px);
                v.y = ra.C > 1 ? __ldg(px + cstride) : 0.f;
                v.z = ra.C > 2 ? __ldg(px + 2 * cstride) : 0.f;
                v.w = ra.C > 3 ? __ldg(px + 3 * cstride) : 0.f;
                return yy * TC_HALO_PITCH + xx;
            };

            for (int gi = 0; gi < P.n_hidden; ++gi) {
                const int buf = (int)(gcount & 1);
                float4 hv = make_float4(0.f, 0.f, 0.f, 0.f);
                const int hslot = halo_fetch(gi * TC_EPI_THREADS + et, hv);
                tr.ev(0xA00 + gi);
                mbar_wait(bar_accfull(buf), (afphase >> buf) & 1);
                afphase ^= 1u << buf;
                tc_fence_after_sync();
                tr.ev(0xB00 + gi);
                const bool need_lo = terms_of(gi + 1) >= 2;
                const uint32_t t_acc = t_lane + buf * 256;
                uint32_t rr[2][32], rf[2][16];
                if (fine) {
                    tmem_ld16(t_acc + hh * 16, rf[0]);
                    tmem_ld16(t_acc + 32 + hh * 16, rf[1]);
                } else {
                    tmem_ld32(t_acc + hh * 32, rr[0]);
                }
#pragma unroll
                for (int j = 0; j < 4; ++j) {
                    tmem_ld_wait();
                    if (j < 3) tmem_ld32(t_acc + (j + 1) * 64 + hh * 32, rr[(j + 1) & 1]);
                    if (j == 0 && fine) {
#pragma unroll
                        for (int c = 0; c < 2; ++c) {
                            const int col = c * 32 + hh * 16;
#pragma unroll
                            for (int i = 0; i < 2; ++i)
                                epi_group8(&rf[c][i * 8], a_hi, a_lo, col / 8 + i, a_row, need_lo);
                            fence_proxy_async_smem();
                            __syncwarp();
                            if (lane == 0) mbar_arrive(bar_aready(c));
                        }
                    } else {
                        const int col = j * 64 + hh * 32;
#pragma unroll
                        for (int i = 0; i < 4; ++i)
                            epi_group8(&rr[j & 1][i * 8], a_hi, a_lo, col / 8 + i, a_row, need_lo);
                        fence_proxy_async_smem();
                        __syncwarp();
                        if (lane == 0) mbar_arrive(bar_aready(fine ? (j == 1 ? 2 : 4) : j));
                    }
                    tr.ev(0xC00 + j);
                }
                tc_fence_before_sync();
                __syncwarp();
                if (lane == 0) mbar_arrive(bar_accfree(buf));
                if (hslot >= 0) s_halo[hslot] = hv;
                ++gcount;
            }
            for (int idx = P.n_hidden * TC_EPI_THREADS + et; !PRED && !dummy && idx < HH * HW; idx += TC_EPI_THREADS) {
                float4 hv;
                const int hslot = halo_fetch(idx, hv);
                s_halo[hslot] = hv;
            }
            named_bar_sync(1, TC_EPI_THREADS);

            float ssum = 0.f, cacc[TC_MAX_C] = {0.f, 0.f, 0.f, 0.f};
            const float4* hbase = s_halo + ty * TC_HALO_PITCH + tx;
            for (int gi = P.n_hidden; gi < P.n_groups; ++gi) {
                const int buf = (int)(gcount & 1);
                tr.ev(0xA00 + gi);
                mbar_wait(bar_accfull(buf), (afphase >> buf) & 1);
                afphase ^= 1u << buf;
                tc_fence_after_sync();
                tr.ev(0xB00 + gi);
                if (gi == P.n_groups - 1 && iter + 1 < my_iters) {
                    layer0(tile + gridDim.x);
                    tr.ev(0x900);
                }
                const int gN = P.g[gi].N, gtap0 = P.g[gi].tap0;
                const float* bias = s_bias + (P.g[gi].bias_off - P.bias_skip);
                if constexpr (PRED) {
                    if (pred_one_block) {
                        float keep[2][32];
#pragma unroll
                        for (int ci = 0; ci < 2; ++ci) {
                            const int c32 = hh * 32 + ci * 64;
                            if (c32 < gN) {
                                uint32_t rr[32];
                                tmem_ld32(t_lane + buf * 256 + c32, rr);
                                const int nvalid = kk - (gtap0 + c32);
                                tmem_ld_wait();
#pragma unroll
                                for (int u = 0; u < 32; ++u) {
                                    float sg = rcp_approx(1.0f + ex2_approx(fmaf(__uint_as_float(rr[u]), NEG_LOG2E, bias[c32 + u])));
                                    sg = (u < nvalid) ? sg : 0.f;
                                    keep[ci][u] = sg;
                                    ssum += sg;
                                }
                            } else {
#pragma unroll
                                for (int u = 0; u < 32; ++u) keep[ci][u] = 0.f;
                            }
                        }
                        tc_fence_before_sync();
                        __syncwarp();
                        if (lane == 0) mbar_arrive(bar_accfree(buf));
                        ++gcount;
                        s_red[row * 5 + hh] = ssum;
                        named_bar_sync(2 + q, 64);
                        const float inv = 1.0f / fmaxf(s_red[row * 5] + s_red[row * 5 + 1], 1e-12f);
                        float* stg = reinterpret_cast<float*>(s_halo) + e * (32 * 9);
                        const long long row0 = tile * TC_M + q * 32;
                        const int rsub = lane >> 3, csub = lane & 7;
#pragma unroll
                        for (int ci = 0; ci < 2; ++ci) {
#pragma unroll
                            for (int pc = 0; pc < 4; ++pc) {
                                const int c0 = gtap0 + hh * 32 + ci * 64 + pc * 8;
                                if (c0 >= kk) continue;
#pragma unroll
                                for (int j = 0; j < 8; ++j) stg[lane * 9 + j] = keep[ci][pc * 8 + j] * inv;
                                __syncwarp();
#pragma unroll
                                for (int rb = 0; rb < 8; ++rb) {
                                    const int rloc = rb * 4 + rsub;
                                    const float v = stg[rloc * 9 + csub];
                                    if (row0 + rloc < P.n_probes && c0 + csub < kk)
                                        P.psf_out[(row0 + rloc) * kk + c0 + csub] = v;
                                }
                                __syncwarp();
                            }
                        }
                        continue;
                    }
                }
#pragma unroll 1
                for (int c32 = hh * 32; c32 < gN; c32 += 64) {
                    uint32_t rr[32];
                    tmem_ld32(t_lane + buf * 256 + c32, rr);
                    const int tap_first = gtap0 + c32;
                    int i = tap_first / ks, j = tap_first - i * ks;
                    int off = i * TC_HALO_PITCH + j;
                    const int nvalid = kk - tap_first;
                    tmem_ld_wait();
                    if constexpr (PRED) {
                        float sgv[32];
#pragma unroll
                        for (int u = 0; u < 32; ++u) {
                            float sg = rcp_approx(1.0f + ex2_approx(fmaf(__uint_as_float(rr[u]), NEG_LOG2E, bias[c32 + u])));
                            sg = (u < nvalid) ? sg : 0.f;
                            sgv[u] = sg;
                            ssum += sg;
                        }
                        float* stg = reinterpret_cast<float*>(s_halo) + e * (32 * 9);
                        const long long row0 = tile * TC_M + q * 32;
                        const int rsub = lane >> 3, csub = lane & 7;
#pragma unroll
                        for (int pc = 0; pc < 4; ++pc) {
                            const int c0 = tap_first + pc * 8;
                            if (c0 >= kk) continue;
#pragma unroll
                            for (int j = 0; j < 8; ++j) stg[lane * 9 + j] = sgv[pc * 8 + j];
                            __syncwarp();
#pragma unroll
                            for (int rb = 0; rb < 8; ++rb) {
                                const int rloc = rb * 4 + rsub;
                                const float v = stg[rloc * 9 + csub];
                                if (row0 + rloc < P.n_probes && c0 + csub < kk) P.psf_out[(row0 + rloc) * kk + c0 + csub] = v;
                            }
                            __syncwarp();
                        }
                    } else if (nvalid >= 32) {
#pragma unroll
                        for (int u = 0; u < 32; ++u) {
                            const float sg = rcp_approx(1.0f + ex2_approx(fmaf(__uint_as_float(rr[u]), NEG_LOG2E, bias[c32 + u])));
                            const float4 px = hbase[off];
                            ssum += sg;
                            cacc[0] = fmaf(sg, px.x, cacc[0]);
                            cacc[1] = fmaf(sg, px.y, cacc[1]);
                            cacc[2] = fmaf(sg, px.z, cacc[2]);
                            cacc[3] = fmaf(sg, px.w, cacc[3]);
                            ++off;
                            if (++j == ks) { j = 0; off += TC_HALO_PITCH - ks; }
                        }
                    } else {
#pragma unroll
                        for (int u = 0; u < 32; ++u) {
                            const bool ok = u < nvalid;
                            float sg = rcp_approx(1.0f + ex2_approx(fmaf(__uint_as_float(rr[u]), NEG_LOG2E, bias[c32 + u])));
                            sg = ok ? sg : 0.f;
                            const float4 px = hbase[ok ? off : 0];
                            ssum += sg;
                            cacc[0] = fmaf(sg, px.x, cacc[0]);
                            cacc[1] = fmaf(sg, px.y, cacc[1]);
                            cacc[2] = fmaf(sg, px.z, cacc[2]);
                            cacc[3] = fmaf(sg, px.w, cacc[3]);
                            ++off;
                            if (++j == ks) { j = 0; off += TC_HALO_PITCH - ks; }
                        }
                    }
                }
                tc_fence_before_sync();
                __syncwarp();
                if (lane == 0) mbar_arrive(bar_accfree(buf));
                ++gcount;
            }
            if constexpr (PRED) {
                if (pred_one_block) continue;
                s_red[row * 5 + hh] = ssum;
                named_bar_sync(2 + q, 64);
                for (int rloc = hh * 16; rloc < hh * 16 + 16; ++rloc) {
                    const long long grow = tile * TC_M + q * 32 + rloc;
                    if (grow >= P.n_probes) break;
                    const float inv = 1.0f / fmaxf(s_red[(q * 32 + rloc) * 5] + s_red[(q * 32 + rloc) * 5 + 1], 1e-12f);
                    float* orow = P.psf_out + grow * kk;
                    for (int t = lane; t < kk; t += 32) orow[t] *= inv;
                }
                continue;
            }
            if (hh == 1) {
                s_red[row * 5 + 0] = ssum;
#pragma unroll
                for (int c = 0; c < TC_MAX_C; ++c) s_red[row * 5 + 1 + c] = cacc[c];
            }
            tr.ev(0xD00);
            named_bar_sync(2 + q, 64);
            if (hh == 0 && valid) {
                const float inv = 1.0f / fmaxf(ssum + s_red[row * 5], 1e-12f);
                float* o = ra.out + n * ra.os_n + ra.c0 * ra.os_c + s * ra.os_s + h * ra.os_h + w * ra.os_w;
#pragma unroll
                for (int c = 0; c < TC_MAX_C; ++c)
                    if (c < ra.C) o[c * ra.os_c] = (cacc[c] + s_red[row * 5 + 1 + c]) * inv;
            }
        }
    }

    tc_fence_before_sync();
    __syncthreads();
    if (CL2) cluster_sync_all();
    if (warp == TC_WARP_PRODUCER) tmem_dealloc<512>(tmem_base);
}

__global__ void __launch_bounds__(128, 1)
debug_umma_gemm_kernel(const float* __restrict__ A, const uint8_t* __restrict__ bpack, float* __restrict__ D,
                       int K, int N, uint32_t swap) {
    extern __shared__ __align__(1024) uint8_t smem[];
    const uint32_t sbase = smem_u32(smem);
    const int warp = threadIdx.x >> 5, lane = threadIdx.x & 31;
    const uint32_t a_hi = sbase;
    const uint32_t b_sm = sbase + TC_A_PART_BYTES;
    const uint32_t bar = sbase + TC_A_PART_BYTES + 131072;
    volatile uint32_t* slot = reinterpret_cast<volatile uint32_t*>(smem + TC_A_PART_BYTES + 131072 + 16);
    if (threadIdx.x == 0) { mbar_init(bar, 1); fence_mbar_init(); }
    if (warp == 0) tmem_alloc<256>(smem_u32(const_cast<uint32_t*>(slot)));
    const int row = threadIdx.x;
    for (int kg = 0; kg < K / 8; ++kg) {
        float v[8];
#pragma unroll
        for (int u = 0; u < 8; ++u) v[u] = A[(size_t)row * K + kg * 8 + u];
        store_split8(v, a_hi + kg * TC_A_LBO + row * 16, 0, false);
    }
    const int bbytes = (K / 32) * N * 64;
    for (int i = threadIdx.x * 16; i < bbytes; i += 128 * 16)
        *reinterpret_cast<uint4*>(smem + TC_A_PART_BYTES + i) = *reinterpret_cast<const uint4*>(bpack + i);
    fence_proxy_async_smem();
    tc_fence_before_sync();
    __syncthreads();
    tc_fence_after_sync();
    const uint32_t tmem_base = *slot;
    if (threadIdx.x == 0) {
        const uint32_t idesc = umma_idesc_f16_f32(128, N);
        const uint32_t lbo_b = (uint32_t)N * 16;
        for (int ks16 = 0; ks16 < K / 16; ++ks16) {
            const uint32_t slab = b_sm + (ks16 / 2) * (N * 64);
            umma_f16_ss(tmem_base, tc_desc(a_hi + ks16 * 2 * TC_A_LBO, TC_A_LBO, 128, swap),
                        tc_desc(slab + (ks16 & 1) * 2 * lbo_b, lbo_b, 128, swap), idesc, ks16 > 0);
        }
        umma_commit(bar);
    }
    __syncwarp();
    mbar_wait(bar, 0);
    tc_fence_after_sync();
    for (int c0 = 0; c0 < N; c0 += 32) {
        uint32_t rr[32];
        tmem_ld32(tmem_base + ((uint32_t)(warp * 32) << 16) + c0, rr);
        tmem_ld_wait();
        for (int u = 0; u < 32; ++u)
            if (c0 + u < N) D[(size_t)row * N + c0 + u] = __uint_as_float(rr[u]);
    }
    tc_fence_before_sync();
    __syncthreads();
    if (warp == 0) tmem_dealloc<256>(tmem_base);
}


__global__ void __launch_bounds__(128, 1)
debug_mma_timing_kernel(unsigned long long* out, int n_patterns, const int* mmas_per_commit, int reps, int N,
                        int epi_load, const uint8_t* __restrict__ gsrc) {
    extern __shared__ __align__(1024) uint8_t smem[];
    const uint32_t sbase = smem_u32(smem);
    const int warp = threadIdx.x >> 5, lane = threadIdx.x & 31;
    const uint32_t a_sm = sbase, b_sm = sbase + TC_A_PART_BYTES;
    const uint32_t bar_done = sbase + TC_A_PART_BYTES + 65536, bar_slab = bar_done + 8;
    volatile uint32_t* slot = reinterpret_cast<volatile uint32_t*>(smem + TC_A_PART_BYTES + 65536 + 32);
    for (int i = threadIdx.x; i < (TC_A_PART_BYTES + 65536) / 4; i += 128) reinterpret_cast<uint32_t*>(smem)[i] = 0;
    const int tmem_reads = epi_load & 0xFFFF;
    const bool do_copy = (epi_load >> 16) & 1, do_sts = (epi_load >> 17) & 1;
    const uint32_t bar_copy = bar_done + 64;
    volatile uint32_t* stop = slot + 1;
    if (threadIdx.x == 0) {
        mbar_init(bar_done, 1); mbar_init(bar_slab, 1);
        for (int i = 0; i < 4; ++i) mbar_init(bar_copy + 8 * i, 1);
        fence_mbar_init();
    }
    if (warp == 0) tmem_alloc<512>(smem_u32(const_cast<uint32_t*>(slot)));
    fence_proxy_async_smem();
    tc_fence_before_sync();
    __syncthreads();
    tc_fence_after_sync();
    const uint32_t tmem_base = *slot;
    uint32_t done_phase = 0, cph = 0;
    for (int p = 0; p < n_patterns; ++p) {
        const int m = mmas_per_commit[p];
        if (threadIdx.x == 0) *stop = 0;
        __syncthreads();
        if (warp == 0) {
            const uint32_t idesc = umma_idesc_f16_f32(128, N);
            const uint64_t da = umma_smem_desc(a_sm, TC_A_LBO, 128);
            const uint64_t db = umma_smem_desc(b_sm, (uint32_t)N * 16, 128);
            const long long t0 = clock64();
            for (int r = 0; r < reps; ++r) {
                if (elect_one_sync()) {
                    for (int i = 0; i < m; ++i)
                        umma_f16_ss(tmem_base, da + (uint32_t)((r * m + i) & 15) * 256u,
                                    db + (uint32_t)(i & 1) * (uint32_t)(2 * N), idesc, 1);
                    umma_commit(bar_slab);
                }
                __syncwarp();
            }
            if (elect_one_sync()) umma_commit(bar_done);
            __syncwarp();
            const long long t1 = clock64();
            mbar_wait(bar_done, done_phase);
            const long long t2 = clock64();
            if (lane == 0) { out[p * 2] = t1 - t0; out[p * 2 + 1] = t2 - t0; *stop = 1; }
        } else if (warp == 1 && do_copy) {
            unsigned long long n = 0;
            if (lane == 0) {
                for (int i = 0; i < 3; ++i) {
                    mbar_arrive_expect_tx(bar_copy + 8 * i, 16384);
                    bulk_g2s(b_sm + 16384 + 16384 * i, gsrc + 16384 * i, 16384, bar_copy + 8 * i);
                }
                while (!*stop) {
                    for (int i = 0; i < 3; ++i) {
                        mbar_wait(bar_copy + 8 * i, (cph >> i) & 1);
                        cph ^= 1u << i;
                        mbar_arrive_expect_tx(bar_copy + 8 * i, 16384);
                        bulk_g2s(b_sm + 16384 + 16384 * i, gsrc + 16384 * i, 16384, bar_copy + 8 * i);
                        ++n;
                    }
                }
                for (int i = 0; i < 3; ++i) {
                    mbar_wait(bar_copy + 8 * i, (cph >> i) & 1);
                    cph ^= 1u << i;
                }
                out[32 + p] = n * 16384ull;
            }
            __syncwarp();
        } else if (warp >= 2 && do_sts) {
            unsigned long long n = 0;
            const uint32_t dst = a_sm + 32768 + (uint32_t)(threadIdx.x - 64) * 16;
            while (!*stop) {
#pragma unroll
                for (int i = 0; i < 8; ++i)
                    asm volatile("st.shared.v4.u32 [%0], {%1,%1,%1,%1};" :: "r"(dst + (uint32_t)i * 1024u), "r"(0u) : "memory");
                n += 8;
            }
            if (threadIdx.x == 64) out[48 + p] = n * 64ull * 16ull;
        } else if (tmem_reads) {
            uint32_t rr[32];
            for (int it = 0; it < tmem_reads; ++it) {
                tmem_ld32(tmem_base + ((uint32_t)(warp * 32) << 16) + 256 + (it & 7) * 32, rr);
                tmem_ld_wait();
            }
            if (rr[0] == 0x12345678u) out[63] = rr[1];
        }
        done_phase ^= 1;
        tc_fence_before_sync();
        __syncthreads();
        tc_fence_after_sync();
    }
    if (warp == 0) tmem_dealloc<512>(tmem_base);
}

}
```

### aberration-aware-depth-from-focus_b200/csrc/ptx_sm100.cuh

```cuda
#pragma once
#include <cstdint>
#include <cuda_runtime.h>

namespace aadff {

__device__ __forceinline__ uint32_t smem_u32(const void* p) {
    return static_cast<uint32_t>(__cvta_generic_to_shared(p));
}

__device__ __forceinline__ void mbar_init(uint32_t bar, uint32_t count) {
    asm volatile("mbarrier.init.shared::cta.b64 [%0], %1;" ::"r"(bar), "r"(count) : "memory");
}
__device__ __forceinline__ void fence_mbar_init() {
    asm volatile("fence.mbarrier_init.release.cluster;" ::: "memory");
}
__device__ __forceinline__ void mbar_arrive(uint32_t bar) {
    asm volatile("mbarrier.arrive.shared::cta.b64 _, [%0];" ::"r"(bar) : "memory");
}
__device__ __forceinline__ void mbar_arrive_expect_tx(uint32_t bar, uint32_t bytes) {
    asm volatile("mbarrier.arrive.expect_tx.shared::cta.b64 _, [%0], %1;" ::"r"(bar), "r"(bytes) : "memory");
}
__device__ __forceinline__ bool mbar_try_wait(uint32_t bar, uint32_t parity) {
    uint32_t ok;
    asm volatile(
        "{\n\t"
        ".reg .pred p;\n\t"
        "mbarrier.try_wait.parity.shared::cta.b64 p, [%1], %2;\n\t"
        "selp.u32 %0, 1, 0, p;\n\t"
        "}"
        : "=r"(ok)
        : "r"(bar), "r"(parity)
        : "memory");
    return ok != 0;
}
__device__ __forceinline__ bool mbar_test_wait(uint32_t bar, uint32_t parity) {
    uint32_t ok;
    asm volatile(
        "{\n\t"
        ".reg .pred p;\n\t"
        "mbarrier.test_wait.parity.shared::cta.b64 p, [%1], %2;\n\t"
        "selp.u32 %0, 1, 0, p;\n\t"
        "}"
        : "=r"(ok)
        : "r"(bar), "r"(parity)
        : "memory");
    return ok != 0;
}
__device__ __forceinline__ void mbar_wait(uint32_t bar, uint32_t parity) {
    while (!mbar_try_wait(bar, parity)) {
    }
}

__device__ __forceinline__ void fence_proxy_async_smem() {
    asm volatile("fence.proxy.async.shared::cta;" ::: "memory");
}
__device__ __forceinline__ void tc_fence_before_sync() {
    asm volatile("tcgen05.fence::before_thread_sync;" ::: "memory");
}
__device__ __forceinline__ void tc_fence_after_sync() {
    asm volatile("tcgen05.fence::after_thread_sync;" ::: "memory");
}

__device__ __forceinline__ void cp_async4(uint32_t dst_smem, const void* src) {
    asm volatile("cp.async.ca.shared.global [%0], [%1], 4;" ::"r"(dst_smem), "l"(src) : "memory");
}
__device__ __forceinline__ void cp_async_wait_all() {
    asm volatile("cp.async.wait_all;" ::: "memory");
}

__device__ __forceinline__ void bulk_g2s(uint32_t dst_smem, const void* src, uint32_t bytes, uint32_t bar) {
    asm volatile(
        "cp.async.bulk.shared::cluster.global.mbarrier::complete_tx::bytes [%0], [%1], %2, [%3];" ::"r"(dst_smem),
        "l"(src), "r"(bytes), "r"(bar)
        : "memory");
}

__device__ __forceinline__ void bulk_g2s_multicast(uint32_t dst_smem, const void* src, uint32_t bytes, uint32_t bar,
                                                   uint16_t cta_mask) {
    asm volatile(
        "cp.async.bulk.shared::cluster.global.mbarrier::complete_tx::bytes.multicast::cluster [%0], [%1], %2, [%3], %4;" ::"r"(
            dst_smem),
        "l"(src), "r"(bytes), "r"(bar), "h"(cta_mask)
        : "memory");
}
__device__ __forceinline__ uint32_t cluster_ctarank() {
    uint32_t r;
    asm volatile("mov.u32 %0, %%cluster_ctarank;" : "=r"(r));
    return r;
}
__device__ __forceinline__ void cluster_sync_all() {
    asm volatile("barrier.cluster.arrive.release.aligned;\n\tbarrier.cluster.wait.acquire.aligned;" ::: "memory");
}

template <int COLS>
__device__ __forceinline__ void tmem_alloc(uint32_t slot_smem) {
    asm volatile("tcgen05.alloc.cta_group::1.sync.aligned.shared::cta.b32 [%0], %1;" ::"r"(slot_smem), "n"(COLS)
                 : "memory");
    asm volatile("tcgen05.relinquish_alloc_permit.cta_group::1.sync.aligned;" ::: "memory");
}
template <int COLS>
__device__ __forceinline__ void tmem_dealloc(uint32_t taddr) {
    asm volatile("tcgen05.dealloc.cta_group::1.sync.aligned.b32 %0, %1;" ::"r"(taddr), "n"(COLS) : "memory");
}

__device__ __forceinline__ void tmem_ld32(uint32_t taddr, uint32_t (&r)[32]) {
    asm volatile(
        "tcgen05.ld.sync.aligned.32x32b.x32.b32 "
        "{%0,%1,%2,%3,%4,%5,%6,%7,%8,%9,%10,%11,%12,%13,%14,%15,"
        "%16,%17,%18,%19,%20,%21,%22,%23,%24,%25,%26,%27,%28,%29,%30,%31}, [%32];"
        : "=r"(r[0]), "=r"(r[1]), "=r"(r[2]), "=r"(r[3]), "=r"(r[4]), "=r"(r[5]), "=r"(r[6]), "=r"(r[7]),
          "=r"(r[8]), "=r"(r[9]), "=r"(r[10]), "=r"(r[11]), "=r"(r[12]), "=r"(r[13]), "=r"(r[14]), "=r"(r[15]),
          "=r"(r[16]), "=r"(r[17]), "=r"(r[18]), "=r"(r[19]), "=r"(r[20]), "=r"(r[21]), "=r"(r[22]), "=r"(r[23]),
          "=r"(r[24]), "=r"(r[25]), "=r"(r[26]), "=r"(r[27]), "=r"(r[28]), "=r"(r[29]), "=r"(r[30]), "=r"(r[31])
        : "r"(taddr)
        : "memory");
}
__device__ __forceinline__ void tmem_ld16(uint32_t taddr, uint32_t (&r)[16]) {
    asm volatile(
        "tcgen05.ld.sync.aligned.32x32b.x16.b32 "
        "{%0,%1,%2,%3,%4,%5,%6,%7,%8,%9,%10,%11,%12,%13,%14,%15}, [%16];"
        : "=r"(r[0]), "=r"(r[1]), "=r"(r[2]), "=r"(r[3]), "=r"(r[4]), "=r"(r[5]), "=r"(r[6]), "=r"(r[7]),
          "=r"(r[8]), "=r"(r[9]), "=r"(r[10]), "=r"(r[11]), "=r"(r[12]), "=r"(r[13]), "=r"(r[14]), "=r"(r[15])
        : "r"(taddr)
        : "memory");
}
__device__ __forceinline__ void tmem_ld_wait() {
    asm volatile("tcgen05.wait::ld.sync.aligned;" ::: "memory");
}

__device__ __forceinline__ uint64_t umma_smem_desc(uint32_t saddr, uint32_t lbo_bytes, uint32_t sbo_bytes) {
    uint64_t d = 0;
    d |= static_cast<uint64_t>((saddr & 0x3FFFFu) >> 4);
    d |= static_cast<uint64_t>((lbo_bytes >> 4) & 0x3FFFu) << 16;
    d |= static_cast<uint64_t>((sbo_bytes >> 4) & 0x3FFFu) << 32;
    d |= static_cast<uint64_t>(1) << 46;
    return d;
}

__host__ __device__ constexpr uint32_t umma_idesc_f16_f32(int M, int N) {
    return (1u << 4) | (static_cast<uint32_t>(N >> 3) << 17) | (static_cast<uint32_t>(M >> 4) << 24);
}

__device__ __forceinline__ void umma_f16_ss(uint32_t d_tmem, uint64_t adesc, uint64_t bdesc, uint32_t idesc,
                                            uint32_t accumulate) {
    asm volatile(
        "{\n\t"
        ".reg .pred p;\n\t"
        "setp.ne.b32 p, %4, 0;\n\t"
        "tcgen05.mma.cta_group::1.kind::f16 [%0], %1, %2, %3, p;\n\t"
        "}" ::"r"(d_tmem),
        "l"(adesc), "l"(bdesc), "r"(idesc), "r"(accumulate)
        : "memory");
}

__device__ __forceinline__ void umma_commit(uint32_t bar) {
    asm volatile("tcgen05.commit.cta_group::1.mbarrier::arrive::one.shared::cluster.b64 [%0];" ::"r"(bar) : "memory");
}

__device__ __forceinline__ void umma_commit_multicast(uint32_t bar, uint16_t cta_mask) {
    asm volatile("tcgen05.commit.cta_group::1.mbarrier::arrive::one.shared::cluster.multicast::cluster.b64 [%0], %1;" ::"r"(bar),
                 "h"(cta_mask)
                 : "memory");
}

__device__ __forceinline__ bool elect_one_sync() {
    uint32_t pred;
    asm volatile(
        "{\n\t"
        ".reg .pred p;\n\t"
        "elect.sync _|p, 0xFFFFFFFF;\n\t"
        "selp.u32 %0, 1, 0, p;\n\t"
        "}"
        : "=r"(pred));
    return pred != 0;
}
__device__ __forceinline__ void named_bar_sync(uint32_t id, uint32_t nthreads) {
    asm volatile("bar.sync %0, %1;" ::"r"(id), "r"(nthreads) : "memory");
}
__device__ __forceinline__ float ex2_approx(float x) {
    float y;
    asm("ex2.approx.ftz.f32 %0, %1;" : "=f"(y) : "f"(x));
    return y;
}
__device__ __forceinline__ float rcp_approx(float x) {
    float y;
    asm("rcp.approx.ftz.f32 %0, %1;" : "=f"(y) : "f"(x));
    return y;
}
__device__ __forceinline__ void st_shared_v4(uint32_t addr, uint32_t a, uint32_t b, uint32_t c, uint32_t d) {
    asm volatile("st.shared.v4.b32 [%0], {%1,%2,%3,%4};" ::"r"(addr), "r"(a), "r"(b), "r"(c), "r"(d) : "memory");
}

}
```

Before: 475.4.

## Feed MMA A operands from tensor memory and defer head gather across tiles

Adds a TA kernel variant where each hidden layer's activations are split into fp16 hi/lo, written to tensor memory with tcgen05.st, and consumed as the A operand of tcgen05.mma (the .kind::f16 form with a TMEM A operand) instead of going through shared memory. The head output is staged to shared memory, and the sigmoid/PSF gather for a tile is deferred so it overlaps the next tile's layer-0 and MMA work. Halo buffers are double-buffered and the shared memory layout is recomputed. This aims to cut shared memory traffic and proxy fences in the epilogue, and to hide gather latency. The cost is extra accumulator-to-accumulator dependencies, since the MMA must wait for the other buffer, plus more complex barrier bookkeeping.

```diff
diff --git a/aberration-aware-depth-from-focus_b200/csrc/aadff_api.cu b/aberration-aware-depth-from-focus_b200/csrc/aadff_api.cu
--- a/aberration-aware-depth-from-focus_b200/csrc/aadff_api.cu
+++ b/aberration-aware-depth-from-focus_b200/csrc/aadff_api.cu
@@ -516,6 +516,10 @@
 #undef AADFF_SET_ATTR
         CREATE_TRY(cudaFuncSetAttribute(fused_psfnet_render_kernel<false, false, 14>, attr, so));
         CREATE_TRY(cudaFuncSetAttribute(fused_psfnet_render_kernel<false, true, 14>, attr, so));
+        CREATE_TRY(cudaFuncSetAttribute(fused_psfnet_render_kernel<true, false, 0, false, true>, attr, so));
+        CREATE_TRY(cudaFuncSetAttribute(fused_psfnet_render_kernel<false, false, 12, false, true>, attr, so));
+        CREATE_TRY(cudaFuncSetAttribute(fused_psfnet_render_kernel<false, false, 13, false, true>, attr, so));
+        CREATE_TRY(cudaFuncSetAttribute(fused_psfnet_render_kernel<false, false, 14, false, true>, attr, so));
     }
 #undef CREATE_TRY
     *out = h;
@@ -711,6 +715,28 @@
     else if (econ8_pat && aligned && h->n_groups > TC_ECON8_FIRST_GROUP) uni = 14;
     else if (mixed_pat && aligned) uni = 15;
     const bool cl2 = P.probes == nullptr && P.trace == nullptr && uni != 0 && uni != 14 && (P.dbg & 8u) && h->num_sms >= 2;
+    bool all2 = true;
+    for (int i = 0; i < h->n_groups; ++i) all2 &= (P.g[i].terms >= 2);
+    const uint32_t head_n = h->groups[h->n_hidden].N;
+    uint32_t smem_launch = smem;
+    const bool ta = P.probes == nullptr && !cl2 && !(P.dbg & (1u << 20)) && h->n_groups == h->n_hidden + 1 &&
+                    h->n_hidden >= 2 && head_n <= (uint32_t)TC_TA_L1_COL && P.kslab == 1 && P.n_stages == 4 && all2 &&
+                    (uni == 12 || uni == 13 || uni == 14 || P.trace != nullptr);
+    if (ta) {
+        const uint32_t stg_bytes = ((head_n + 31u) & ~31u) * TC_M * 4;
+        P.halo_bytes = halo_bytes;
+        P.off_stage = 0;
+        P.off_stg = 4 * TC_STAGE_BYTES;
+        P.off_bias = P.off_stg + stg_bytes;
+        P.off_w0 = P.off_bias + bias_bytes;
+        P.off_halo = (P.off_w0 + 320 * 4 + 15u) & ~15u;
+        P.off_red = P.off_halo + 2 * halo_bytes;
+        P.off_bar = P.off_red + TC_M * 5 * 4;
+        P.off_ones = (P.off_bar + TC_BAR_BYTES + 15u) & ~15u;
+        P.off_bslab = P.off_ones + ones_bytes;
+        smem_launch = P.off_bslab + bslab_bytes;
+        if (smem_launch > (uint32_t)h->smem_optin) return fail(AADFF_E_UNSUPPORTED, "shared memory budget exceeded (TA)");
+    }
     if (cl2) {
         grid = (int)std::min<long long>((P.n_tiles + 1) & ~1ll, (long long)(h->num_sms & ~1));
         cudaLaunchConfig_t cfg{};
@@ -733,7 +759,14 @@
         }
         if (le != cudaSuccess) return fail(AADFF_E_CUDA, std::string("cluster launch: ") + cudaGetErrorString(le));
     } else if (P.trace != nullptr && P.probes == nullptr) {
-        fused_psfnet_render_kernel<true, false, 0><<<grid, TC_NT, smem, st>>>(P);
+        if (ta) fused_psfnet_render_kernel<true, false, 0, false, true><<<grid, TC_NT, smem_launch, st>>>(P);
+        else fused_psfnet_render_kernel<true, false, 0><<<grid, TC_NT, smem, st>>>(P);
+    } else if (ta) {
+        switch (uni) {
+            case 12: fused_psfnet_render_kernel<false, false, 12, false, true><<<grid, TC_NT, smem_launch, st>>>(P); break;
+            case 13: fused_psfnet_render_kernel<false, false, 13, false, true><<<grid, TC_NT, smem_launch, st>>>(P); break;
+            default: fused_psfnet_render_kernel<false, false, 14, false, true><<<grid, TC_NT, smem_launch, st>>>(P); break;
+        }
     } else {
 #define AADFF_LAUNCH(U)                                                                                   \
         case U:                                                                                           \
diff --git a/aberration-aware-depth-from-focus_b200/csrc/fused_tc_kernel.cuh b/aberration-aware-depth-from-focus_b200/csrc/fused_tc_kernel.cuh
--- a/aberration-aware-depth-from-focus_b200/csrc/fused_tc_kernel.cuh
+++ b/aberration-aware-depth-from-focus_b200/csrc/fused_tc_kernel.cuh
@@ -28,6 +28,8 @@
 constexpr int TC_MIXED_FIRST_GROUP = 3;
 constexpr int TC_ECON_FIRST_GROUP = 4;
 constexpr int TC_ECON8_FIRST_GROUP = 7;
+constexpr int TC_TA_L1_COL = TC_HID - 64;
+constexpr int TC_TA_L1_BAR = 5;
 
 struct TcGroup {
     uint32_t w_off;
@@ -54,6 +56,8 @@
     long long tile0;
     uint32_t off_stage, off_bias, off_w0, off_halo, off_red, off_bar, off_ones;
     uint32_t off_bslab;
+    uint32_t off_stg;
+    uint32_t halo_bytes;
     uint32_t dbg;
     const float* probes;
     float* psf_out;
@@ -138,12 +142,36 @@
     st_shared_v4(a_lo + off, l[0], l[1], l[2], l[3]);
 }
 
+__device__ __forceinline__ void epi_ta16(const uint32_t* acc, uint32_t taddr) {
+    uint32_t o[16];
+#pragma unroll
+    for (int u = 0; u < 8; ++u) {
+        const float a0 = __uint_as_float(acc[2 * u]), a1 = __uint_as_float(acc[2 * u + 1]);
+        o[u] = pack_half2_relu_rz(a0, a1);
+        const float2 f = __half22float2(*reinterpret_cast<__half2*>(&o[u]));
+        o[8 + u] = pack_half2_relu(a0 - f.x, a1 - f.y);
+    }
+    tmem_st16(taddr, o);
+}
+
+__device__ __forceinline__ void split_ta16(const float (&v)[16], uint32_t taddr) {
+    uint32_t o[16];
+#pragma unroll
+    for (int u = 0; u < 8; ++u) {
+        o[u] = pack_half2(v[2 * u], v[2 * u + 1]);
+        const float2 f = __half22float2(*reinterpret_cast<__half2*>(&o[u]));
+        o[8 + u] = pack_half2(v[2 * u] - f.x, v[2 * u + 1] - f.y);
+    }
+    tmem_st16(taddr, o);
+}
+
 constexpr int TC_WARP_PRODUCER = TC_EPI_WARPS;
 constexpr int TC_WARP_MMA = TC_EPI_WARPS + 1;
 
-template <bool TRACE, bool PRED, int UNI, bool CL2 = false>
+template <bool TRACE, bool PRED, int UNI, bool CL2 = false, bool TA = false>
 __global__ void __launch_bounds__(TC_NT, 1) fused_psfnet_render_kernel(const __grid_constant__ TcParams P) {
     static_assert(!(CL2 && (PRED || TRACE)), "the cluster variant exists for the render kernels only");
+    static_assert(!(TA && (CL2 || PRED)), "tensor-memory A operands exist for the one-CTA render kernels only");
     constexpr int UM = UNI % 10;
     const uint32_t cta_rank = CL2 ? cluster_ctarank() : 0u;
     const long long first_tile = CL2 ? (long long)(blockIdx.x & ~1u) : (long long)blockIdx.x;
@@ -184,7 +212,8 @@
     if (threadIdx.x == 0) {
         for (int s = 0; s < TC_MAX_STAGES; ++s) { mbar_init(bar_full(s), 1); mbar_init(bar_empty(s), CL2 ? 2 : 1); }
         for (int j = 0; j < 8; ++j)
-            mbar_init(bar_aready(j), (kslab_c == 2 || j < 4) ? TC_EPI_WARPS : 2 * TC_EPI_WARPS);
+            mbar_init(bar_aready(j), (kslab_c == 2 || j < 4 || (TA && (j == TC_TA_L1_BAR || j == TC_TA_L1_BAR + 1)))
+                                         ? TC_EPI_WARPS : 2 * TC_EPI_WARPS);
         for (int b = 0; b < 2; ++b) { mbar_init(bar_accfull(b), 1); mbar_init(bar_accfree(b), TC_EPI_WARPS); }
         mbar_init(bar_bfull(), 1);
         mbar_init(bar_bempty(), 1);
@@ -269,6 +298,7 @@
         int stage = 0;
         uint32_t fbits = 0, aphase = 0, frphase = 0;
         uint32_t bphase = 0;
+        uint32_t afbits = 0;
         uint32_t gcount = 0;
         TcTrace<TRACE> tr; tr.init(lane == 0 ? P.trace : nullptr, 1);
         const uint64_t da_hi = umma_smem_desc(a_hi, TC_A_LBO, 128);
@@ -292,9 +322,15 @@
                     mbar_wait(bar_accfree(buf), (frphase >> buf) & 1);
                     frphase ^= 1u << buf;
                 }
+                if (TA && gcount >= 1) {
+                    mbar_wait(bar_accfull(buf ^ 1), (afbits >> (buf ^ 1)) & 1);
+                    afbits ^= 1u << (buf ^ 1);
+                }
                 tc_fence_after_sync();
                 tr.ev(0x200 + gi);
                 const uint32_t d_tmem = tmem_base + buf * 256;
+                const uint32_t a_tmem = tmem_base + (buf ^ 1) * 256 + (gi == 0 ? TC_TA_L1_COL : 0);
+                const int abar0 = (TA && gi == 0) ? TC_TA_L1_BAR : 0;
                 const uint32_t idesc = umma_idesc_f16_f32(TC_M, gN);
                 const uint32_t kstep_b = (2 * gN * 16) >> 4;
                 const uint64_t db0 = umma_smem_desc(stage0, gN * 16, 128);
@@ -316,14 +352,18 @@
                     const int kc = it * kslab;
                     const uint64_t ah = da_hi + (uint32_t)kc * (2 * KSTEP_A);
                     const uint64_t al = da_lo + (uint32_t)kc * (2 * KSTEP_A);
+                    auto mma_a = [&](bool lo, int k16, uint64_t b, uint32_t acc) {
+                        if constexpr (TA) umma_f16_ts(d_tmem, a_tmem + (uint32_t)(kc * 32 + k16 * 16 + (lo ? 8 : 0)), b, idesc, acc);
+                        else umma_f16_ss(d_tmem, (lo ? al : ah) + (uint32_t)k16 * KSTEP_A, b, idesc, acc);
+                    };
                     if (ALIGNED) stage = (three ? 2 * it : it) & 3;
                     if (!pre_waited) {
                         tr.ev(0x500 + kc);
                         { mbar_wait(bar_full(stage), (fbits >> stage) & 1); fbits ^= 1u << stage; }
                         tr.ev(0x600 + kc);
                         if (new_a && (kslab == 2 || it < 3 || it == 4)) {
-                            mbar_wait(bar_aready(it), (aphase >> it) & 1);
-                            aphase ^= 1u << it;
+                            mbar_wait(bar_aready(abar0 + it), (aphase >> (abar0 + it)) & 1);
+                            aphase ^= 1u << (abar0 + it);
                             tr.ev(0x400 + kc);
                         }
                     }
@@ -336,10 +376,10 @@
                         const bool merged = three && (ALIGNED || P.n_stages >= 4);
                         if (elect_one_sync()) {
                             const uint64_t db = (db0 & ~0x3FFFull) | ((stage_addr(hi_stage) & 0x3FFFFu) >> 4);
-                            umma_f16_ss(d_tmem, ah, db, idesc, has_bias || it != 0);
-                            umma_f16_ss(d_tmem, ah + KSTEP_A, db + kstep_b, idesc, 1);
-                            umma_f16_ss(d_tmem, al, db, idesc, 1);
-                            umma_f16_ss(d_tmem, al + KSTEP_A, db + kstep_b, idesc, 1);
+                            mma_a(false, 0, db, has_bias || it != 0);
+                            mma_a(false, 1, db + kstep_b, 1);
+                            mma_a(true, 0, db, 1);
+                            mma_a(true, 1, db + kstep_b, 1);
                             if (!three) {
                                 if (last) umma_commit(bar_accfull(buf));
                                 release(bar_empty(hi_stage));
@@ -347,8 +387,8 @@
                                 release(bar_empty(hi_stage));
                                 if (merged) {
                                     const uint64_t dl = (db0 & ~0x3FFFull) | ((stage_addr(stage) & 0x3FFFFu) >> 4);
-                                    umma_f16_ss(d_tmem, ah, dl, idesc, 1);
-                                    umma_f16_ss(d_tmem, ah + KSTEP_A, dl + kstep_b, idesc, 1);
+                                    mma_a(false, 0, dl, 1);
+                                    mma_a(false, 1, dl + kstep_b, 1);
                                     if (last) umma_commit(bar_accfull(buf));
                                     release(bar_empty(stage));
                                 }
@@ -361,8 +401,8 @@
                                 tc_fence_after_sync();
                                 if (elect_one_sync()) {
                                     const uint64_t dl = (db0 & ~0x3FFFull) | ((stage_addr(stage) & 0x3FFFFu) >> 4);
-                                    umma_f16_ss(d_tmem, ah, dl, idesc, 1);
-                                    umma_f16_ss(d_tmem, ah + KSTEP_A, dl + kstep_b, idesc, 1);
+                                    mma_a(false, 0, dl, 1);
+                                    mma_a(false, 1, dl + kstep_b, 1);
                                     if (last) umma_commit(bar_accfull(buf));
                                     release(bar_empty(stage));
                                 }
@@ -374,11 +414,11 @@
                     }
                     if (elect_one_sync()) {
                         const uint64_t db = (db0 & ~0x3FFFull) | ((stage_addr(hi_stage) & 0x3FFFFu) >> 4);
-                        umma_f16_ss(d_tmem, ah, db, idesc, has_bias || it != 0);
-                        umma_f16_ss(d_tmem, ah + KSTEP_A, db + kstep_b, idesc, 1);
+                        mma_a(false, 0, db, has_bias || it != 0);
+                        mma_a(false, 1, db + kstep_b, 1);
                         if (kslab == 2) {
-                            umma_f16_ss(d_tmem, ah + 2 * KSTEP_A, db + STAGE_STEP, idesc, 1);
-                            umma_f16_ss(d_tmem, ah + 3 * KSTEP_A, db + STAGE_STEP + kstep_b, idesc, 1);
+                            mma_a(false, 2, db + STAGE_STEP, 1);
+                            mma_a(false, 3, db + STAGE_STEP + kstep_b, 1);
                         }
                     }
                     __syncwarp();
@@ -388,8 +428,8 @@
                         tr.ev(0x500 + kc + kslab);
                         { mbar_wait(bar_full(stage), (fbits >> stage) & 1); fbits ^= 1u << stage; }
                         if (new_a && (kslab == 2 || it + 1 < 3 || it + 1 == 4)) {
-                            mbar_wait(bar_aready(it + 1), (aphase >> (it + 1)) & 1);
-                            aphase ^= 1u << (it + 1);
+                            mbar_wait(bar_aready(abar0 + it + 1), (aphase >> (abar0 + it + 1)) & 1);
+                            aphase ^= 1u << (abar0 + it + 1);
                         }
                         tr.ev(0x400 + kc + kslab);
                         pre_waited = true;
@@ -461,7 +501,7 @@
         float nx_depth = 0.f, nx_foc = 0.f;
         fetch_dz(blockIdx.x, nx_depth, nx_foc);
 
-        auto layer0 = [&](long long t) {
+        auto layer0 = [&](long long t, uint32_t ta_buf) {
             float x, y, z, fz;
             if constexpr (PRED) {
                 x = nx_in.x; y = nx_in.y; z = nx_in.z; fz = nx_in.w;
@@ -473,6 +513,27 @@
                 z = depth_to_z(nx_depth, ra.d_min, ra.d_range);
                 fz = depth_to_z(nx_foc, ra.d_min, ra.d_range);
             }
+            if constexpr (TA) {
+#pragma unroll
+                for (int st = 0; st < 2; ++st) {
+                    const int k16 = 2 * st + hh;
+                    float v[16];
+#pragma unroll
+                    for (int u = 0; u < 16; ++u) {
+                        const int f = k16 * 16 + u;
+                        const float4 wv = *reinterpret_cast<const float4*>(s_w0 + f * 4);
+                        float a = s_w0[256 + f];
+                        a = fmaf(wv.x, x, a); a = fmaf(wv.y, y, a); a = fmaf(wv.z, z, a); a = fmaf(wv.w, fz, a);
+                        v[u] = fmaxf(a, 0.f);
+                    }
+                    split_ta16(v, t_lane + ta_buf * 256 + TC_TA_L1_COL + k16 * 16);
+                }
+                tmem_st_wait();
+                tc_fence_before_sync();
+                __syncwarp();
+                if (lane == 0) { mbar_arrive(bar_aready(TC_TA_L1_BAR)); mbar_arrive(bar_aready(TC_TA_L1_BAR + 1)); }
+                return;
+            }
             const bool need_lo = terms_of(0) >= 2;
 #pragma unroll
             for (int i = 0; i < 4; ++i) {
@@ -496,7 +557,82 @@
                 else mbar_arrive(bar_aready(0));
             }
         };
-        if (my_iters > 0) layer0(blockIdx.x);
+        if (my_iters > 0) layer0(blockIdx.x, 1u);
+
+        auto gather32 = [&](const uint32_t (&rr)[32], int tap_first, const float* bias_c, const float4* hbase, float& ssum,
+                            float (&cacc)[TC_MAX_C]) {
+            int i = tap_first / ks, j = tap_first - i * ks;
+            int off = i * TC_HALO_PITCH + j;
+            const int nvalid = kk - tap_first;
+            if (nvalid >= 32) {
+#pragma unroll
+                for (int u = 0; u < 32; ++u) {
+                    const float sg = rcp_approx(1.0f + ex2_approx(fmaf(__uint_as_float(rr[u]), NEG_LOG2E, bias_c[u])));
+                    const float4 px = hbase[off];
+                    ssum += sg;
+                    cacc[0] = fmaf(sg, px.x, cacc[0]);
+                    cacc[1] = fmaf(sg, px.y, cacc[1]);
+                    cacc[2] = fmaf(sg, px.z, cacc[2]);
+                    cacc[3] = fmaf(sg, px.w, cacc[3]);
+                    ++off;
+                    if (++j == ks) { j = 0; off += TC_HALO_PITCH - ks; }
+                }
+            } else {
+#pragma unroll
+                for (int u = 0; u < 32; ++u) {
+                    const bool ok = u < nvalid;
+                    float sg = rcp_approx(1.0f + ex2_approx(fmaf(__uint_as_float(rr[u]), NEG_LOG2E, bias_c[u])));
+                    sg = ok ? sg : 0.f;
+                    const float4 px = hbase[ok ? off : 0];
+                    ssum += sg;
+                    cacc[0] = fmaf(sg, px.x, cacc[0]);
+                    cacc[1] = fmaf(sg, px.y, cacc[1]);
+                    cacc[2] = fmaf(sg, px.z, cacc[2]);
+                    cacc[3] = fmaf(sg, px.w, cacc[3]);
+                    ++off;
+                    if (++j == ks) { j = 0; off += TC_HALO_PITCH - ks; }
+                }
+            }
+        };
+        auto store_px = [&](float ssum, const float (&cacc)[TC_MAX_C], int n, int s, int h, int w, bool valid) {
+            if (hh == 1) {
+                s_red[row * 5 + 0] = ssum;
+#pragma unroll
+                for (int c = 0; c < TC_MAX_C; ++c) s_red[row * 5 + 1 + c] = cacc[c];
+            }
+            tr.ev(0xD00);
+            named_bar_sync(2 + q, 64);
+            if (hh == 0 && valid) {
+                const float inv = 1.0f / fmaxf(ssum + s_red[row * 5], 1e-12f);
+                float* o = ra.out + n * ra.os_n + ra.c0 * ra.os_c + s * ra.os_s + h * ra.os_h + w * ra.os_w;
+#pragma unroll
+                for (int c = 0; c < TC_MAX_C; ++c)
+                    if (c < ra.C) o[c * ra.os_c] = (cacc[c] + s_red[row * 5 + 1 + c]) * inv;
+            }
+        };
+
+        const int halo_f4 = (int)(P.halo_bytes / 16);
+        auto gather_ta = [&](long long piter) {
+            int pn, ps, h0, w0;
+            tile_coords(blockIdx.x + piter * gridDim.x, pn, ps, h0, w0);
+            float ssum = 0.f, cacc[TC_MAX_C] = {0.f, 0.f, 0.f, 0.f};
+            const float4* hbase = s_halo + (piter & 1) * halo_f4 + ty * TC_HALO_PITCH + tx;
+            const float4* stg = reinterpret_cast<const float4*>(smem + P.off_stg) + row;
+            const int gi = P.n_hidden;
+            const float* bias = s_bias + (P.g[gi].bias_off - P.bias_skip);
+#pragma unroll 1
+            for (int c32 = hh * 32; c32 < P.g[gi].N; c32 += 64) {
+                uint32_t rr[32];
+#pragma unroll
+                for (int k = 0; k < 8; ++k) {
+                    const float4 v = stg[(c32 / 4 + k) * TC_M];
+                    rr[4 * k] = __float_as_uint(v.x); rr[4 * k + 1] = __float_as_uint(v.y);
+                    rr[4 * k + 2] = __float_as_uint(v.z); rr[4 * k + 3] = __float_as_uint(v.w);
+                }
+                gather32(rr, P.g[gi].tap0 + c32, bias + c32, hbase, ssum, cacc);
+            }
+            store_px(ssum, cacc, pn, ps, h0 + ty, w0 + tx, (h0 + ty < ra.H) && (w0 + tx < ra.W));
+        };
 
         long long tile = blockIdx.x;
         for (long long iter = 0; iter < my_iters; ++iter, tile += gridDim.x) {
@@ -509,7 +645,8 @@
             tr.ev(0x800);
             fetch_dz(tile + gridDim.x, nx_depth, nx_foc);
 
-            named_bar_sync(1, TC_EPI_THREADS);
+            if (!TA) named_bar_sync(1, TC_EPI_THREADS);
+            float4* const s_halo_t = s_halo + (TA ? (int)(iter & 1) * halo_f4 : 0);
             const float* img_n = ra.img + ((long long)n * ra.Ctot + ra.c0) * ra.H * ra.W;
             const long long cstride = (long long)ra.H * ra.W;
             auto halo_fetch = [&](int idx, float4& v) -> int {
@@ -536,53 +673,114 @@
                 const bool need_lo = terms_of(gi + 1) >= 2;
                 const uint32_t t_acc = t_lane + buf * 256;
                 uint32_t rr[2][32], rf[2][16];
-                if (fine) {
+                if constexpr (TA) {
                     tmem_ld16(t_acc + hh * 16, rf[0]);
                     tmem_ld16(t_acc + 32 + hh * 16, rf[1]);
+#pragma unroll
+                    for (int j = 0; j < 4; ++j) {
+                        tmem_ld_wait();
+                        if (j < 3) tmem_ld32(t_acc + (j + 1) * 64 + hh * 32, rr[(j + 1) & 1]);
+                        if (j == 0) {
+#pragma unroll
+                            for (int c = 0; c < 2; ++c) {
+                                epi_ta16(rf[c], t_acc + c * 32 + hh * 16);
+                                tmem_st_wait();
+                                tc_fence_before_sync();
+                                __syncwarp();
+                                if (lane == 0) mbar_arrive(bar_aready(c));
+                            }
+                        } else {
+                            const int col = j * 64 + hh * 32;
+                            epi_ta16(&rr[j & 1][0], t_acc + col);
+                            epi_ta16(&rr[j & 1][16], t_acc + col + 16);
+                            tmem_st_wait();
+                            tc_fence_before_sync();
+                            __syncwarp();
+                            if (lane == 0) mbar_arrive(bar_aready(j == 1 ? 2 : 4));
+                        }
+                        tr.ev(0xC00 + j);
+                    }
                 } else {
-                    tmem_ld32(t_acc + hh * 32, rr[0]);
-                }
-#pragma unroll
-                for (int j = 0; j < 4; ++j) {
-                    tmem_ld_wait();
-                    if (j < 3) tmem_ld32(t_acc + (j + 1) * 64 + hh * 32, rr[(j + 1) & 1]);
-                    if (j == 0 && fine) {
-#pragma unroll
-                        for (int c = 0; c < 2; ++c) {
-                            const int col = c * 32 + hh * 16;
-#pragma unroll
-                            for (int i = 0; i < 2; ++i)
-                                epi_group8(&rf[c][i * 8], a_hi, a_lo, col / 8 + i, a_row, need_lo);
+                    if (fine) {
+                        tmem_ld16(t_acc + hh * 16, rf[0]);
+                        tmem_ld16(t_acc + 32 + hh * 16, rf[1]);
+                    } else {
+                        tmem_ld32(t_acc + hh * 32, rr[0]);
+                    }
+#pragma unroll
+                    for (int j = 0; j < 4; ++j) {
+                        tmem_ld_wait();
+                        if (j < 3) tmem_ld32(t_acc + (j + 1) * 64 + hh * 32, rr[(j + 1) & 1]);
+                        if (j == 0 && fine) {
+#pragma unroll
+                            for (int c = 0; c < 2; ++c) {
+                                const int col = c * 32 + hh * 16;
+#pragma unroll
+                                for (int i = 0; i < 2; ++i)
+                                    epi_group8(&rf[c][i * 8], a_hi, a_lo, col / 8 + i, a_row, need_lo);
+                                fence_proxy_async_smem();
+                                __syncwarp();
+                                if (lane == 0) mbar_arrive(bar_aready(c));
+                            }
+                        } else {
+                            const int col = j * 64 + hh * 32;
+#pragma unroll
+                            for (int i = 0; i < 4; ++i)
+                                epi_group8(&rr[j & 1][i * 8], a_hi, a_lo, col / 8 + i, a_row, need_lo);
                             fence_proxy_async_smem();
                             __syncwarp();
-                            if (lane == 0) mbar_arrive(bar_aready(c));
-                        }
-                    } else {
-                        const int col = j * 64 + hh * 32;
-#pragma unroll
-                        for (int i = 0; i < 4; ++i)
-                            epi_group8(&rr[j & 1][i * 8], a_hi, a_lo, col / 8 + i, a_row, need_lo);
-                        fence_proxy_async_smem();
-                        __syncwarp();
-                        if (lane == 0) mbar_arrive(bar_aready(fine ? (j == 1 ? 2 : 4) : j));
-                    }
-                    tr.ev(0xC00 + j);
+                            if (lane == 0) mbar_arrive(bar_aready(fine ? (j == 1 ? 2 : 4) : j));
+                        }
+                        tr.ev(0xC00 + j);
+                    }
                 }
                 tc_fence_before_sync();
                 __syncwarp();
                 if (lane == 0) mbar_arrive(bar_accfree(buf));
-                if (hslot >= 0) s_halo[hslot] = hv;
+                if (hslot >= 0) s_halo_t[hslot] = hv;
                 ++gcount;
+                if constexpr (TA) {
+                    if (gi == 0 && iter > 0) gather_ta(iter - 1);
+                    if (gi == P.n_hidden - 1 && iter + 1 < my_iters) {
+                        layer0(tile + gridDim.x, (uint32_t)(gcount & 1));
+                        tr.ev(0x900);
+                    }
+                }
             }
             for (int idx = P.n_hidden * TC_EPI_THREADS + et; !PRED && !dummy && idx < HH * HW; idx += TC_EPI_THREADS) {
                 float4 hv;
                 const int hslot = halo_fetch(idx, hv);
-                s_halo[hslot] = hv;
+                s_halo_t[hslot] = hv;
             }
             named_bar_sync(1, TC_EPI_THREADS);
 
+            if constexpr (TA) {
+                const int buf = (int)(gcount & 1), gi = P.n_hidden;
+                tr.ev(0xA00 + gi);
+                mbar_wait(bar_accfull(buf), (afphase >> buf) & 1);
+                afphase ^= 1u << buf;
+                tc_fence_after_sync();
+                tr.ev(0xB00 + gi);
+                float4* stg = reinterpret_cast<float4*>(smem + P.off_stg) + row;
+#pragma unroll 1
+                for (int c32 = hh * 32; c32 < P.g[gi].N; c32 += 64) {
+                    uint32_t rr[32];
+                    tmem_ld32(t_lane + buf * 256 + c32, rr);
+                    tmem_ld_wait();
+#pragma unroll
+                    for (int k = 0; k < 8; ++k)
+                        stg[(c32 / 4 + k) * TC_M] = make_float4(__uint_as_float(rr[4 * k]), __uint_as_float(rr[4 * k + 1]),
+                                                                __uint_as_float(rr[4 * k + 2]), __uint_as_float(rr[4 * k + 3]));
+                }
+                tc_fence_before_sync();
+                __syncwarp();
+                if (lane == 0) mbar_arrive(bar_accfree(buf));
+                ++gcount;
+                continue;
+            }
+
             float ssum = 0.f, cacc[TC_MAX_C] = {0.f, 0.f, 0.f, 0.f};
-            const float4* hbase = s_halo + ty * TC_HALO_PITCH + tx;
+            const float4* hbase = s_halo_t + ty * TC_HALO_PITCH + tx;
             for (int gi = P.n_hidden; gi < P.n_groups; ++gi) {
                 const int buf = (int)(gcount & 1);
                 tr.ev(0xA00 + gi);
@@ -591,7 +789,7 @@
                 tc_fence_after_sync();
                 tr.ev(0xB00 + gi);
                 if (gi == P.n_groups - 1 && iter + 1 < my_iters) {
-                    layer0(tile + gridDim.x);
+                    layer0(tile + gridDim.x, 0u);
                     tr.ev(0x900);
                 }
                 const int gN = P.g[gi].N, gtap0 = P.g[gi].tap0;
@@ -656,11 +854,9 @@
                     uint32_t rr[32];
                     tmem_ld32(t_lane + buf * 256 + c32, rr);
                     const int tap_first = gtap0 + c32;
-                    int i = tap_first / ks, j = tap_first - i * ks;
-                    int off = i * TC_HALO_PITCH + j;
-                    const int nvalid = kk - tap_first;
                     tmem_ld_wait();
                     if constexpr (PRED) {
+                        const int nvalid = kk - tap_first;
                         float sgv[32];
 #pragma unroll
                         for (int u = 0; u < 32; ++u) {
@@ -687,34 +883,8 @@
                             }
                             __syncwarp();
                         }
-                    } else if (nvalid >= 32) {
-#pragma unroll
-                        for (int u = 0; u < 32; ++u) {
-                            const float sg = rcp_approx(1.0f + ex2_approx(fmaf(__uint_as_float(rr[u]), NEG_LOG2E, bias[c32 + u])));
-                            const float4 px = hbase[off];
-                            ssum += sg;
-                            cacc[0] = fmaf(sg, px.x, cacc[0]);
-                            cacc[1] = fmaf(sg, px.y, cacc[1]);
-                            cacc[2] = fmaf(sg, px.z, cacc[2]);
-                            cacc[3] = fmaf(sg, px.w, cacc[3]);
-                            ++off;
-                            if (++j == ks) { j = 0; off += TC_HALO_PITCH - ks; }
-                        }
                     } else {
-#pragma unroll
-                        for (int u = 0; u < 32; ++u) {
-                            const bool ok = u < nvalid;
-                            float sg = rcp_approx(1.0f + ex2_approx(fmaf(__uint_as_float(rr[u]), NEG_LOG2E, bias[c32 + u])));
-                            sg = ok ? sg : 0.f;
-                            const float4 px = hbase[ok ? off : 0];
-                            ssum += sg;
-                            cacc[0] = fmaf(sg, px.x, cacc[0]);
-                            cacc[1] = fmaf(sg, px.y, cacc[1]);
-                            cacc[2] = fmaf(sg, px.z, cacc[2]);
-                            cacc[3] = fmaf(sg, px.w, cacc[3]);
-                            ++off;
-                            if (++j == ks) { j = 0; off += TC_HALO_PITCH - ks; }
-                        }
+                        gather32(rr, tap_first, bias + c32, hbase, ssum, cacc);
                     }
                 }
                 tc_fence_before_sync();
@@ -735,20 +905,10 @@
                 }
                 continue;
             }
-            if (hh == 1) {
-                s_red[row * 5 + 0] = ssum;
-#pragma unroll
-                for (int c = 0; c < TC_MAX_C; ++c) s_red[row * 5 + 1 + c] = cacc[c];
-            }
-            tr.ev(0xD00);
-            named_bar_sync(2 + q, 64);
-            if (hh == 0 && valid) {
-                const float inv = 1.0f / fmaxf(ssum + s_red[row * 5], 1e-12f);
-                float* o = ra.out + n * ra.os_n + ra.c0 * ra.os_c + s * ra.os_s + h * ra.os_h + w * ra.os_w;
-#pragma unroll
-                for (int c = 0; c < TC_MAX_C; ++c)
-                    if (c < ra.C) o[c * ra.os_c] = (cacc[c] + s_red[row * 5 + 1 + c]) * inv;
-            }
+            store_px(ssum, cacc, n, s, h, w, valid);
+        }
+        if constexpr (TA) {
+            if (my_iters > 0) gather_ta(my_iters - 1);
         }
     }
 
diff --git a/aberration-aware-depth-from-focus_b200/csrc/ptx_sm100.cuh b/aberration-aware-depth-from-focus_b200/csrc/ptx_sm100.cuh
--- a/aberration-aware-depth-from-focus_b200/csrc/ptx_sm100.cuh
+++ b/aberration-aware-depth-from-focus_b200/csrc/ptx_sm100.cuh
@@ -127,6 +127,17 @@
 __device__ __forceinline__ void tmem_ld_wait() {
     asm volatile("tcgen05.wait::ld.sync.aligned;" ::: "memory");
 }
+__device__ __forceinline__ void tmem_st16(uint32_t taddr, const uint32_t (&r)[16]) {
+    asm volatile(
+        "tcgen05.st.sync.aligned.32x32b.x16.b32 [%0], "
+        "{%1,%2,%3,%4,%5,%6,%7,%8,%9,%10,%11,%12,%13,%14,%15,%16};" ::"r"(taddr),
+        "r"(r[0]), "r"(r[1]), "r"(r[2]), "r"(r[3]), "r"(r[4]), "r"(r[5]), "r"(r[6]), "r"(r[7]),
+        "r"(r[8]), "r"(r[9]), "r"(r[10]), "r"(r[11]), "r"(r[12]), "r"(r[13]), "r"(r[14]), "r"(r[15])
+        : "memory");
+}
+__device__ __forceinline__ void tmem_st_wait() {
+    asm volatile("tcgen05.wait::st.sync.aligned;" ::: "memory");
+}
 
 __device__ __forceinline__ uint64_t umma_smem_desc(uint32_t saddr, uint32_t lbo_bytes, uint32_t sbo_bytes) {
     uint64_t d = 0;
@@ -153,6 +164,18 @@
         : "memory");
 }
 
+__device__ __forceinline__ void umma_f16_ts(uint32_t d_tmem, uint32_t a_tmem, uint64_t bdesc, uint32_t idesc,
+                                            uint32_t accumulate) {
+    asm volatile(
+        "{\n\t"
+        ".reg .pred p;\n\t"
+        "setp.ne.b32 p, %4, 0;\n\t"
+        "tcgen05.mma.cta_group::1.kind::f16 [%0], [%1], %2, %3, p;\n\t"
+        "}" ::"r"(d_tmem),
+        "r"(a_tmem), "l"(bdesc), "r"(idesc), "r"(accumulate)
+        : "memory");
+}
+
 __device__ __forceinline__ void umma_commit(uint32_t bar) {
     asm volatile("tcgen05.commit.cta_group::1.mbarrier::arrive::one.shared::cluster.b64 [%0];" ::"r"(bar) : "memory");
 }
```

Measured after the change: 496.1, median of 6. +4.4%, better.
